# Gaurav14cs17/Bayer_Low_light_Image_Enhancement

Measured on AMD Instinct MI355X. Metric: megapixels/sec RawFormer-S 512x512 RAW->sRGB, higher is better.
Workload: dtype f32; 1 GPU; RawFormer-S(FLCA) dim=32, batch=8 of packed 4x512x512 synthetic Bayer per GPU; frames_per_gpu=8, variant=flca, weights=synthetic (seeded, random-init scale), parallelism=batch-sharded x1, device=AMD Radeon Graphics

## Files before the change

### bayer_low_light_image_enhancement_amd/build.py

```python
from __future__ import annotations

import os
import shutil
import subprocess
import sys
import tempfile
from concurrent.futures import ThreadPoolExecutor

HERE = os.path.dirname(os.path.abspath(__file__))
CSRC = os.path.join(HERE, "csrc")
LIB = os.path.join(CSRC, "librawformer_hip.so")
DIAG_LIB = os.path.join(CSRC, "librawformer_hip_diag.so")
DIAG_SOURCES = ["rf_block.hip", "rf_model.hip", "rf_gemm1x1.hip", "rf_fused.hip"]
SOURCES = ["rf_api.hip", "rf_model.hip", "rf_pack.hip", "rf_pointwise.hip", "rf_gemm1x1.hip",
           "rf_conv3x3.hip", "rf_attn.hip", "rf_flca.hip", "rf_fused.hip", "rf_block.hip", "rf_harness.hip", "rf_tokattn.hip", "rf_wfb.hip", "rf_upcat.hip", "rf_fft.hip", "rf_ffab.hip", "rf_truecolor.hip", "rf_train.hip", "rf_trainstep.hip"]
HEADERS = [os.path.join(CSRC, "rf_common.h"), os.path.join(CSRC, "rf_handle.h"), os.path.join(HERE, "..", "include", "rawformer_hip.h"),
           os.path.join(HERE, "isa_check.py")]
FLAGS = ["-O3", "-std=c++17", "-fPIC", "--offload-arch=gfx950", "-Wall", "-Wno-unused-function"]


def _hipcc() -> str:
    exe = shutil.which("hipcc") or "/opt/rocm/bin/hipcc"
    if not os.path.exists(exe):
        raise RuntimeError("hipcc not found: the RawFormer HIP library cannot be built here")
    return exe


def _run(cmd, cwd=None) -> str:
    r = subprocess.run(cmd, capture_output=True, text=True, cwd=cwd)
    if r.returncode != 0:
        raise RuntimeError("build step failed:\n" + " ".join(cmd) + "\n" + r.stdout + r.stderr)
    return r.stderr


def compile_source(src: str, obj: str, extra_flags=(), verbose: bool = False) -> int:
    from . import isa_check

    hipcc = _hipcc()
    llvm = isa_check.LLVM_BIN
    flags = [*FLAGS, *extra_flags]
    tmp = tempfile.mkdtemp(prefix="rf_build_")
    try:
        dev_s, dev_o, dev_co, fb = (os.path.join(tmp, n) for n in ("dev.s", "dev.o", "dev.co", "dev.hipfb"))
        warn = _run([hipcc, *flags, "--cuda-device-only", "-S", src, "-o", dev_s])
        text, nfix = isa_check.commute_vulnerable(open(dev_s).read())
        if nfix:
            open(dev_s, "w").write(text)
        _run([os.path.join(llvm, "clang"), "-target", "amdgcn-amd-amdhsa", "-mcpu=gfx950", "-c", dev_s, "-o", dev_o])
        _run([os.path.join(llvm, "lld"), "-flavor", "gnu", "-m", "elf64_amdgpu", "--no-undefined", "-shared", "-o", dev_co, dev_o])
        _run([os.path.join(llvm, "clang-offload-bundler"), "-type=o", "-bundle-align=4096",
              "-targets=host-x86_64-unknown-linux-gnu,hipv4-amdgcn-amd-amdhsa--gfx950", "-input=/dev/null", f"-input={dev_co}", f"-output={fb}"])
        _run([hipcc, *flags, "--cuda-host-only", "-c", src, "-Xclang", "-fcuda-include-gpubinary", "-Xclang", fb, "-o", obj])
    finally:
        shutil.rmtree(tmp, ignore_errors=True)
    if verbose:
        print(f"{os.path.basename(src)}: {nfix} packed-f32 operand-select instruction(s) commuted" + (("\n" + warn) if warn.strip() else ""), flush=True)
    return nfix


def _stale(target: str, deps) -> bool:
    if not os.path.exists(target):
        return True
    t = os.path.getmtime(target)
    return any(os.path.getmtime(d) > t for d in deps)


def build_library(force: bool = False, verbose: bool = False) -> str:
    hipcc = _hipcc()
    headers = HEADERS
    objs, jobs = [], []
    for src in SOURCES:
        s = os.path.join(CSRC, src)
        o = os.path.join(CSRC, src.replace(".hip", ".o"))
        objs.append(o)
        if force or _stale(o, [s] + headers):
            jobs.append((s, o))

    with ThreadPoolExecutor(max_workers=4) as ex:
        list(ex.map(lambda so: compile_source(so[0], so[1], verbose=verbose), jobs))
    if force or jobs or _stale(LIB, objs):
        _run([hipcc, "-shared", "-fPIC", "--offload-arch=gfx950", *objs, "-o", LIB])
    return LIB


def build_diag_library(force: bool = False, verbose: bool = False) -> str:
    build_library(force=force, verbose=verbose)
    hipcc = _hipcc()
    headers = HEADERS
    objs, rebuilt = [], False
    for src in SOURCES:
        s = os.path.join(CSRC, src)
        if src in DIAG_SOURCES:
            o = os.path.join(CSRC, src.replace(".hip", "_diag.o"))
            if force or _stale(o, [s] + headers):
                compile_source(s, o, extra_flags=["-DRF_DIAG"], verbose=verbose)
                rebuilt = True
        else:
            o = os.path.join(CSRC, src.replace(".hip", ".o"))
        objs.append(o)
    if force or rebuilt or _stale(DIAG_LIB, objs):
        r = subprocess.run([hipcc, "-shared", "-fPIC", "--offload-arch=gfx950", *objs, "-o", DIAG_LIB], capture_output=True, text=True)
        if r.returncode != 0:
            raise RuntimeError("hipcc link failed:\n" + r.stdout + r.stderr)
    return DIAG_LIB


if __name__ == "__main__":
    print(build_library(force="--force" in sys.argv, verbose=True))
    if "--diag" in sys.argv:
        print(build_diag_library(verbose=True))
```

### bayer_low_light_image_enhancement_amd/csrc/rf_api.hip

```cpp
#include <cstdarg>
#include <cstdio>
#include <cstring>
#include <map>
#include <string>
#include <vector>
#include "rf_common.h"

namespace rf {

static thread_local char g_err[512] = "";

void set_error(const char* fmt, ...) {
    va_list ap;
    va_start(ap, fmt);
    vsnprintf(g_err, sizeof(g_err), fmt, ap);
    va_end(ap);
}

int check_hip(hipError_t e, const char* what) {
    if (e == hipSuccess) return RF_OK;
    set_error("%s: %s", what, hipGetErrorString(e));
    return RF_E_DEVICE;
}

int check_launch(const char* what) { return check_hip(hipGetLastError(), what); }

struct ProfRec {
    std::string key;
    double flops, bytes;
    hipEvent_t e0, e1;
};
static bool g_prof_on = false;
static std::vector<ProfRec> g_prof;

ProfScope::ProfScope(hipStream_t st, const char* key, double flops, double bytes) : st_(st), rec_(-1) {
    if (!g_prof_on) return;
    ProfRec r;
    r.key = key;
    r.flops = flops;
    r.bytes = bytes;
    if (hipEventCreate(&r.e0) != hipSuccess || hipEventCreate(&r.e1) != hipSuccess) return;
    (void)hipEventRecord(r.e0, st);
    rec_ = (int)g_prof.size();
    g_prof.push_back(r);
}

bool profiling_active() { return g_prof_on; }

ProfScope::~ProfScope() {
    if (rec_ >= 0) (void)hipEventRecord(g_prof[rec_].e1, st_);
}

static const float kHaarInit[16] = {
    0.5f, 0.5f, 0.5f, 0.5f, -0.5f, 0.5f, -0.5f, 0.5f, -0.5f, -0.5f, 0.5f, 0.5f, 0.5f, -0.5f, -0.5f, 0.5f};
static const float kHaarOrtho[16] = {
    0.5f, 0.5f, 0.5f, 0.5f, 0.5f, -0.5f, 0.5f, -0.5f, 0.5f, 0.5f, -0.5f, -0.5f, 0.5f, -0.5f, -0.5f, 0.5f};

}

using namespace rf;

extern "C" {

const char* rf_last_error(void) { return g_err; }
int rf_version(void) { return 1; }

int rf_profile_begin(void) {
    for (auto& r : g_prof) { (void)hipEventDestroy(r.e0); (void)hipEventDestroy(r.e1); }
    g_prof.clear();
    g_prof_on = true;
    return RF_OK;
}

int rf_profile_end(char* json, size_t len) {
    g_prof_on = false;
    struct Agg { long n = 0; double ms = 0, flops = 0, bytes = 0; };
    std::map<std::string, Agg> agg;
    int rc = RF_OK;
    for (auto& r : g_prof) {
        float ms = 0.f;
        if (hipEventSynchronize(r.e1) != hipSuccess || hipEventElapsedTime(&ms, r.e0, r.e1) != hipSuccess) rc = RF_E_DEVICE;
        Agg& a = agg[r.key];
        a.n += 1; a.ms += ms; a.flops += r.flops; a.bytes += r.bytes;
        (void)hipEventDestroy(r.e0);
        (void)hipEventDestroy(r.e1);
    }
    g_prof.clear();
    if (rc) { set_error("rf_profile_end: event timing failed"); return rc; }
    std::string out = "[";
    bool first = true;
    for (auto& kv : agg) {
        char buf[512];
        snprintf(buf, sizeof(buf), "%s{\"kernel\": \"%s\", \"launches\": %ld, \"ms\": %.6f, \"flops\": %.6e, \"bytes\": %.6e}",
                 first ? "" : ", ", kv.first.c_str(), kv.second.n, kv.second.ms, kv.second.flops, kv.second.bytes);
        out += buf;
        first = false;
    }
    out += "]";
    RF_CHECK_ARG(json && out.size() + 1 <= len, "rf_profile_end: buffer of %zu bytes too small (need %zu)", len, out.size() + 1);
    memcpy(json, out.c_str(), out.size() + 1);
    return RF_OK;
}

int rf_pixel_unshuffle2(const float* in, float* out, int B, int C, int h, int w, void* stream) {
    RF_CHECK_ARG(in && out && B > 0 && C > 0 && h > 0 && w > 0, "pixel_unshuffle2: bad arguments");
    return launch_pixel_unshuffle2(in, out, B, C, h, w, (hipStream_t)stream);
}

int rf_pixel_shuffle2(const float* in, float* out, int B, int C, int h, int w, void* stream) {
    RF_CHECK_ARG(in && out && B > 0 && C > 0 && h > 0 && w > 0, "pixel_shuffle2: bad arguments");
    return launch_pixel_shuffle2(in, out, B, C, h, w, (hipStream_t)stream);
}

int rf_dwt_haar(const float* in, float* out, int B, int C, int h, int w, void* stream) {
    RF_CHECK_ARG(in && out && B > 0 && C > 0 && h > 0 && w > 0, "dwt_haar: bad arguments");
    return launch_dwt2x2(in, out, kHaarInit, 0, 1, B, C, h, w, 2 * h, 2 * w, (hipStream_t)stream);
}

int rf_idwt_haar(const float* in, float* out, int B, int C, int h, int w, void* stream) {
    RF_CHECK_ARG(in && out && B > 0 && C > 0 && h > 0 && w > 0, "idwt_haar: bad arguments");
    return launch_idwt2x2(in, out, kHaarInit, 0, 1, B, C, h, w, (hipStream_t)stream);
}

static void scaled_kernel(const float* k16, int norm, float out[16]) {
    for (int i = 0; i < 16; ++i) out[i] = norm ? k16[i] / 2.0f : k16[i];
}

int rf_dwt_custom(const float* in, float* out, const float* k16, int norm, int B, int C, int h, int w, void* stream) {
    RF_CHECK_ARG(in && out && k16 && B > 0 && C > 0 && h > 0 && w > 0, "dwt_custom: bad arguments");
    float k[16];
    scaled_kernel(k16, norm, k);
    return launch_dwt2x2(in, out, k, 1, 0, B, C, h, w, 2 * h, 2 * w, (hipStream_t)stream);
}

int rf_idwt_custom(const float* in, float* out, const float* k16, int norm, int B, int C, int h, int w, void* stream) {
    RF_CHECK_ARG(in && out && k16 && B > 0 && C > 0 && h > 0 && w > 0, "idwt_custom: bad arguments");
    float k[16];
    scaled_kernel(k16, norm, k);
    return launch_idwt2x2(in, out, k, 1, 0, B, C, h, w, (hipStream_t)stream);
}

int rf_haar_dwt(const float* in, float* out, int B, int C, int hin, int win, void* stream) {
    RF_CHECK_ARG(in && out && B > 0 && C > 0 && hin > 1 && win > 1, "haar_dwt: bad arguments");
    return launch_dwt2x2(in, out, kHaarOrtho, 0, 0, B, C, (hin + 1) / 2, (win + 1) / 2, hin, win, (hipStream_t)stream);
}

int rf_layernorm2d(const float* in, float* out, const float* weight, const float* bias, float eps,
                   int B, int C, int h, int w, void* stream) {
    RF_CHECK_ARG(in && out && weight && B > 0 && C > 0 && h > 0 && w > 0, "layernorm2d: bad arguments");
    return launch_layernorm2d(in, out, weight, bias, eps, B, C, h * w, (hipStream_t)stream);
}

int rf_conv1x1_scratch_bytes(int Cin_total, int Cout, size_t* bytes) {
    RF_CHECK_ARG(bytes && Cin_total > 0 && Cout > 0, "conv1x1_scratch_bytes: bad arguments");
    *bytes = (align_up(packed1x1_floats(Cin_total, Cout), 64) + packed1x1_b3_floats(Cin_total, Cout)) * sizeof(float);
    return RF_OK;
}

int rf_conv1x1(const float* in, const float* in2, float* out, const float* weight, const float* bias,
               const float* ln_w, const float* ln_b, const float* res, void* scratch,
               int B, int C1, int C2, int Cout, int h, int w, void* stream) {
    RF_CHECK_ARG(in && out && weight && scratch && aligned16(scratch), "conv1x1: bad arguments");
    hipStream_t st = (hipStream_t)stream;
    const int K = C1 + C2;
    RF_TRY(pack_1x1(weight, (float*)scratch, Cout, K, K, 1, st));
    float* w3 = (float*)scratch + align_up(packed1x1_floats(K, Cout), 64);
    RF_TRY(pack_1x1_b3(weight, w3, Cout, K, K, 1, st));
    Conv1x1Args a{};
    a.x1 = in; a.C1 = C1; a.x1_bstride = (int64_t)C1 * h * w;
    a.x2 = C2 ? in2 : nullptr; a.C2 = C2; a.x2_bstride = (int64_t)C2 * h * w;
    a.wp = (const float*)scratch; a.wp3 = w3; a.bias = bias; a.ln_w = ln_w; a.ln_b = ln_b; a.ln_eps = 1e-5f;
    a.res = res; a.res_bstride = (int64_t)Cout * h * w;
    a.out = out; a.out_bstride = (int64_t)Cout * h * w; a.Cout = Cout; a.B = B; a.P = h * w; a.w = w;
    return launch_conv1x1(a, st);
}

int rf_dwconv3x3(const float* in, float* out, const float* weight, const float* bias, int gelu,
                 int B, int C, int h, int w, void* stream) {
    RF_CHECK_ARG(in && out && weight && B > 0 && C > 0 && h > 0 && w > 0, "dwconv3x3: bad arguments");
    DwConvArgs a{};
    a.x = in; a.x_bstride = (int64_t)C * h * w; a.out = out; a.out_bstride = (int64_t)C * h * w;
    a.w = weight; a.bias = bias; a.B = B; a.C = C; a.h = h; a.w_ = w; a.gelu = gelu;
    return launch_dwconv3x3(a, (hipStream_t)stream);
}

int rf_conv3x3_scratch_bytes(int Cin, int Cout, size_t* bytes) {
    RF_CHECK_ARG(bytes && Cin > 0 && Cout > 0, "conv3x3_scratch_bytes: bad arguments");
    *bytes = packed3x3_floats(Cin, Cout) * sizeof(float);
    return RF_OK;
}

int rf_conv3x3(const float* in, float* out, const float* weight, const float* bias, void* scratch,
               int act, int store, int B, int Cin, int Cout, int h, int w, void* stream) {
    RF_CHECK_ARG(in && out && weight && scratch && aligned16(scratch), "conv3x3: bad arguments");
    hipStream_t st = (hipStream_t)stream;
    RF_TRY(pack_3x3(weight, (float*)scratch, Cout, Cin, st));
    Conv3x3Args a{};
    a.x = in; a.x_bstride = (int64_t)Cin * h * w; a.wp = (const float*)scratch; a.bias = bias;
    a.out = out; a.out_bstride = (int64_t)Cout * h * w; a.B = B; a.Cin = Cin; a.Cout = Cout; a.h = h; a.w = w;
    a.act = act; a.store = store;
    return launch_conv3x3(a, st);
}

int rf_convT2x2_scratch_bytes(int Cin, int Cout, size_t* bytes) {
    RF_CHECK_ARG(bytes && Cin > 0 && Cout > 0, "convT2x2_scratch_bytes: bad arguments");
    *bytes = packed1x1_floats(Cin, 4 * Cout) * sizeof(float);
    return RF_OK;
}

int rf_convT2x2(const float* in, float* out, const float* weight, const float* bias, void* scratch,
                int B, int Cin, int Cout, int h, int w, void* stream) {
    RF_CHECK_ARG(in && out && weight && scratch && aligned16(scratch), "convT2x2: bad arguments");
    hipStream_t st = (hipStream_t)stream;
    RF_TRY(pack_convT(weight, (float*)scratch, Cin, Cout, st));
    Conv1x1Args a{};
    a.x1 = in; a.C1 = Cin; a.x1_bstride = (int64_t)Cin * h * w; a.wp = (const float*)scratch; a.bias = bias;
    a.out = out; a.out_bstride = (int64_t)Cout * 4 * h * w; a.Cout = 4 * Cout; a.B = B; a.P = h * w; a.w = w; a.mode = 1;
    return launch_conv1x1(a, st);
}

struct AttnScratch {
    size_t wqkv, wqkv3, pre, qkv, partial, wfold, wfold3, total;
};
static int attn_scratch(int B, int C, int heads, int h, int w, AttnScratch* s) {
    const int P = h * w;
    int ns, sl;
    size_t pf;
    RF_TRY(gram_plan(B, C, heads, P, &ns, &sl, &pf));
    if (attn_mid_supported(C, heads, h, w)) {
        size_t pf2;
        attn_mid_plan(h, w, &ns, &pf2, B, C);
        if (pf2 > pf) pf = pf2;
    }
    size_t off = 0;
    auto take = [&](size_t f) { const size_t o = off; off += align_up(f, 64); return o; };
    s->wqkv = take(packed1x1_floats(C, 3 * C));
    s->wqkv3 = take(packed1x1_b3_floats(C, 3 * C));
    s->pre = take((size_t)B * 3 * C * P);
    s->qkv = take((size_t)B * 3 * C * P);
    s->partial = take(pf);
    s->wfold = take((size_t)B * packed1x1_floats(C, C));
    s->wfold3 = take((size_t)B * packed1x1_b3_floats(C, C));
    s->total = off;
    return RF_OK;
}

int rf_chan_attn_scratch_bytes(int B, int C, int heads, int h, int w, size_t* bytes) {
    RF_CHECK_ARG(bytes && B > 0 && C > 0 && heads > 0 && h > 0 && w > 0, "chan_attn_scratch_bytes: bad arguments");
    AttnScratch s;
    RF_TRY(attn_scratch(B, C, heads, h, w, &s));
    *bytes = s.total * sizeof(float);
    return RF_OK;
}

int rf_chan_attn(const float* in, float* out, const float* qkv_w, const float* qkv_b,
                 const float* dw_w, const float* dw_b, const float* temperature,
                 const float* proj_w, const float* proj_b, void* scratch,
                 int B, int C, int heads, int h, int w, void* stream) {
    RF_CHECK_ARG(in && out && qkv_w && dw_w && temperature && proj_w && scratch && aligned16(scratch), "chan_attn: bad arguments");
    hipStream_t st = (hipStream_t)stream;
    const int P = h * w;
    AttnScratch s;
    RF_TRY(attn_scratch(B, C, heads, h, w, &s));
    float* ws = (float*)scratch;
    RF_TRY(pack_1x1(qkv_w, ws + s.wqkv, 3 * C, C, C, 1, st));
    RF_TRY(pack_1x1_b3(qkv_w, ws + s.wqkv3, 3 * C, C, C, 1, st));
    Conv1x1Args q{};
    q.x1 = in; q.C1 = C; q.x1_bstride = (int64_t)C * P; q.wp = ws + s.wqkv; q.wp3 = ws + s.wqkv3; q.bias = qkv_b;
    q.out = ws + s.pre; q.out_bstride = (int64_t)3 * C * P; q.Cout = 3 * C; q.B = B; q.P = P; q.w = w;
    RF_TRY(launch_conv1x1(q, st));
    Conv1x1Args av{};
    int nslab = 0;
    if (attn_mid_supported(C, heads, h, w)) {
        size_t pf;
        RF_TRY(attn_mid_plan(h, w, &nslab, &pf, B, C));
        RF_TRY(launch_attn_mid(ws + s.pre, ws + s.qkv, ws + s.partial, nslab, dw_w, dw_b, B, C, h, w, st));
        av.x1 = ws + s.qkv; av.x1_bstride = (int64_t)C * P;
    } else {
        DwConvArgs d{};
        d.x = ws + s.pre; d.x_bstride = (int64_t)3 * C * P; d.out = ws + s.qkv; d.out_bstride = (int64_t)3 * C * P;
        d.w = dw_w; d.bias = dw_b; d.B = B; d.C = 3 * C; d.h = h; d.w_ = w;
        RF_TRY(launch_dwconv3x3(d, st));
        GramArgs g{};
        g.q = ws + s.qkv; g.k = ws + s.qkv + (size_t)C * P; g.bstride = (int64_t)3 * C * P;
        g.B = B; g.C = C; g.heads = heads; g.P = P; g.partial = ws + s.partial;
        size_t pf;
        RF_TRY(gram_plan(B, C, heads, P, &g.nslab, &g.slab, &pf));
        RF_TRY(launch_gram(g, st));
        nslab = g.nslab;
        av.x1 = ws + s.qkv + (size_t)2 * C * P; av.x1_bstride = (int64_t)3 * C * P;
    }
    RF_TRY(launch_attn_fold(ws + s.partial, nslab, temperature, proj_w, ws + s.wfold, ws + s.wfold3, B, C, heads, st));
    av.C1 = C;
    av.wp = ws + s.wfold; av.wp_bstride = (int64_t)packed1x1_floats(C, C); av.bias = proj_b;
    av.wp3 = ws + s.wfold3; av.wp3_bstride = (int64_t)packed1x1_b3_floats(C, C);
    av.out = out; av.out_bstride = (int64_t)C * P; av.Cout = C; av.B = B; av.P = P; av.w = w;
    return launch_conv1x1(av, st);
}

struct TbScratch { size_t wqkv, w1, w2, wqkv3, w13, w23, bufs, total; TbBufOffsets o; };
static void tb_scratch(int B, int C, int heads, int hc, int h, int w, TbScratch* s) {
    size_t off = 0;
    auto take = [&](size_t f) { const size_t r = off; off += align_up(f, 64); return r; };
    s->wqkv = take(packed1x1_floats(C, 3 * C));
    s->w1 = take(packed1x1_floats(C, hc));
    s->w2 = take(packed1x1_floats(hc, C));
    s->wqkv3 = take(packed1x1_b3_floats(C, 3 * C));
    s->w13 = take(packed1x1_b3_floats(C, hc));
    s->w23 = take(packed1x1_b3_floats(hc, C));
    s->bufs = off;
    s->total = off + transformer_scratch_floats(B, C, heads, hc, h, w, &s->o);
}

int rf_transformer_block_scratch_bytes(int B, int C, int heads, int ffn_expansion, int h, int w, size_t* bytes) {
    RF_CHECK_ARG(bytes && B > 0 && C > 0 && heads > 0 && C % heads == 0 && ffn_expansion > 0 && h > 0 && w > 0, "transformer_block_scratch_bytes: bad arguments");
    { int ns, sl; size_t pf; RF_TRY(gram_plan(B, C, heads, h * w, &ns, &sl, &pf)); }
    TbScratch s;
    tb_scratch(B, C, heads, C * ffn_expansion, h, w, &s);
    *bytes = s.total * sizeof(float);
    return RF_OK;
}

int rf_transformer_block(const float* in, float* out, const float* const* prm, void* scratch,
                         int B, int C, int heads, int ffn_expansion, int h, int w, void* stream) {
    RF_CHECK_ARG(in && out && prm && scratch && aligned16(scratch), "transformer_block: bad arguments");
    RF_CHECK_ARG(B > 0 && C % 4 == 0 && heads > 0 && C % heads == 0 && C / heads <= 64, "transformer_block: unsupported C=%d heads=%d", C, heads);
    for (int i = 0; i < 17; ++i) RF_CHECK_ARG(prm[i] != nullptr, "transformer_block: parameter %d is null", i);
    hipStream_t st = (hipStream_t)stream;
    const int hc = C * ffn_expansion;
    { int ns, sl; size_t pf; RF_TRY(gram_plan(B, C, heads, h * w, &ns, &sl, &pf)); }
    TbScratch s;
    tb_scratch(B, C, heads, hc, h, w, &s);
    float* ws = (float*)scratch;
    RF_TRY(pack_1x1(prm[3], ws + s.wqkv, 3 * C, C, C, 1, st));
    RF_TRY(pack_1x1(prm[11], ws + s.w1, hc, C, C, 1, st));
    RF_TRY(pack_1x1(prm[15], ws + s.w2, C, hc, hc, 1, st));
    RF_TRY(pack_1x1_b3(prm[3], ws + s.wqkv3, 3 * C, C, C, 1, st));
    RF_TRY(pack_1x1_b3(prm[11], ws + s.w13, hc, C, C, 1, st));
    RF_TRY(pack_1x1_b3(prm[15], ws + s.w23, C, hc, hc, 1, st));
    TbParams p{prm[0], prm[1], prm[2], ws + s.wqkv, prm[4], prm[5], prm[6], prm[7], prm[8],
               prm[9], prm[10], ws + s.w1, prm[12], prm[13], prm[14], ws + s.w2, prm[16],
               ws + s.wqkv3, ws + s.w13, ws + s.w23, 0};
    return run_transformer(p, in, out, ws + s.bufs, s.o, B, C, heads, hc, h, w, st);
}

int rf_flca_scratch_bytes(int B, int C, int h, int w, size_t* bytes) {
    RF_CHECK_ARG(bytes && B > 0 && C > 0 && h > 0 && w > 0, "flca_scratch_bytes: bad arguments");
    *bytes = (align_up((size_t)B * flca_nblk(h, w) * C, 64) + align_up((size_t)B * C, 64)) * sizeof(float);
    return RF_OK;
}

int rf_flca(const float* feat, const float* guide, float* out, const float* const* prm, void* scratch,
            int B, int C, int h, int w, void* stream) {
    RF_CHECK_ARG(feat && guide && out && prm && scratch && aligned16(scratch), "flca: bad arguments");
    for (int i = 0; i < 10; ++i) RF_CHECK_ARG(prm[i] != nullptr, "flca: parameter %d is null", i);
    hipStream_t st = (hipStream_t)stream;
    float* partial = (float*)scratch;
    float* ch = partial + align_up((size_t)B * flca_nblk(h, w) * C, 64);
    FlcaSpatialArgs a{};
    a.feat = feat; a.xs = out; a.guide = guide;
    a.alpha = prm[0]; a.beta = prm[1]; a.gamma = prm[2]; a.w_low = prm[3]; a.w_high = prm[4]; a.w_chr = prm[5];
    a.partial = partial; a.B = B; a.C = C; a.h = h; a.w = w; a.nblk = flca_nblk(h, w);
    RF_TRY(launch_flca_spatial(a, st));
    const int hid = C / 8 > 8 ? C / 8 : 8;
    RF_TRY(launch_flca_se(partial, a.nblk, h * w, prm[6], prm[7], prm[8], prm[9], hid, ch, B, C, st));
    return launch_scale_channels(out, ch, B, C, h * w, st);
}

int rf_guidance_scratch_bytes(int B, int H, int W, size_t* bytes) {
    RF_CHECK_ARG(bytes && B > 0 && H > 0 && W > 0, "guidance_scratch_bytes: bad arguments");
    *bytes = guidance_scratch_floats(B, H, W) * sizeof(float);
    return RF_OK;
}

int rf_flca_guidance(const float* packed, float* guide, void* scratch, int B, int H, int W, int hf, int wf, void* stream) {
    RF_CHECK_ARG(packed && guide && scratch && hf > 0 && wf > 0, "flca_guidance: bad arguments");
    hipStream_t st = (hipStream_t)stream;
    RF_TRY(launch_guidance_base(packed, 0, 0, (float*)scratch, B, H, W, st));
    return launch_guidance_level((const float*)scratch, guide, B, H, W, hf, wf, st);
}

int rf_upcat_scratch_bytes(int C, size_t* bytes) {
    RF_CHECK_ARG(bytes && C > 0 && C % 4 == 0, "upcat_scratch_bytes: bad arguments");
    *bytes = upcat_packed_floats(C) * sizeof(float);
    return RF_OK;
}

int rf_upcat(const float* x, const float* skip, float* out, const float* up_w, const float* up_b, const float* cr_w, const float* cr_b,
             void* scratch, int B, int C, int h, int w, void* stream) {
    RF_CHECK_ARG(x && skip && out && up_w && cr_w && scratch && aligned16(scratch), "upcat: bad arguments");
    hipStream_t st = (hipStream_t)stream;
    RF_TRY(pack_upcat(up_w, up_b, cr_w, cr_b, (float*)scratch, C, st));
    return launch_upcat(x, skip, out, (const float*)scratch, B, C, h, w, st);
}
}
```

### bayer_low_light_image_enhancement_amd/csrc/rf_common.h

```cpp
#pragma once
#include <hip/hip_runtime.h>
#include <stdint.h>
#include <stddef.h>
#include "../../include/rawformer_hip.h"

namespace rf {

typedef float f32x4 __attribute__((ext_vector_type(4)));

void set_error(const char* fmt, ...);
int check_hip(hipError_t e, const char* what);
int check_launch(const char* what);

#define RF_CHECK_ARG(cond, ...)            \
    do {                                   \
        if (!(cond)) {                     \
            rf::set_error(__VA_ARGS__);    \
            return RF_E_INVALID;           \
        }                                  \
    } while (0)

#define RF_TRY(expr)            \
    do {                        \
        const int rc_ = (expr); \
        if (rc_) return rc_;    \
    } while (0)

struct ProfScope {
    ProfScope(hipStream_t st, const char* key, double flops, double bytes);
    ~ProfScope();
    hipStream_t st_;
    int rec_;
};
bool profiling_active();

__device__ __forceinline__ float gelu_fast(float v) {
    const float t = __builtin_amdgcn_rcpf(fmaf(0.3275911f * 0.70710678118654752440f, fabsf(v), 1.0f));
    float p = fmaf(1.061405429f, t, -1.453152027f);
    p = fmaf(p, t, 1.421413741f);
    p = fmaf(p, t, -0.284496736f);
    p = fmaf(p, t, 0.254829592f);
    const float ex = __builtin_amdgcn_exp2f((v * v) * (-0.5f * 1.44269504088896340736f));
    const float q = (p * t) * ex;
    const float h = 0.5f * v;
    return h + fmaf(-fabsf(h), q, fabsf(h));
}

static inline int cdiv(int a, int b) { return (a + b - 1) / b; }
static inline size_t align_up(size_t v, size_t a) { return (v + a - 1) / a * a; }
static inline bool aligned16(const void* p) { return (reinterpret_cast<uintptr_t>(p) & 15) == 0; }

static inline size_t packed1x1_floats(int K, int Cout) { return (size_t)cdiv(K, 4) * cdiv(Cout, 16) * 64; }
static inline size_t packed3x3_floats(int Cin, int Cout) { return (size_t)cdiv(Cin, 8) * 2 * 18 * cdiv(Cout, 16) * 64; }

static inline size_t packed1x1_b3_floats(int K, int Cout) { return (size_t)cdiv(K, 32) * cdiv(Cout, 16) * 768; }
int pack_1x1_b3(const float* w, void* packed3, int Cout, int K, int64_t row_stride, int64_t col_stride, hipStream_t st);
#ifdef __HIPCC__
typedef unsigned u32x4 __attribute__((ext_vector_type(4)));
typedef __bf16 bf16x8 __attribute__((ext_vector_type(8)));
__device__ __forceinline__ void b3_split(float x, unsigned& p0, unsigned& p1, unsigned& p2) {
    p0 = __float_as_uint(x);
    const float r1 = x - __uint_as_float(p0 & 0xffff0000u);
    p1 = __float_as_uint(r1);
    p2 = __float_as_uint(r1 - __uint_as_float(p1 & 0xffff0000u));
}
__device__ __forceinline__ unsigned b3_pack(unsigned even_elem, unsigned odd_elem) {
    return __builtin_amdgcn_perm(odd_elem, even_elem, 0x07060302u);
}
__device__ __forceinline__ size_t b3_index(int NT, int co, int k, int piece) {
    const int lane = (co & 15) + 16 * ((k & 31) >> 3);
    return ((((size_t)(k >> 5) * NT + (co >> 4)) * 3 + piece) * 64 + lane) * 8 + (k & 7);
}
__device__ __forceinline__ void b3_store(unsigned short* dst, int NT, int co, int k, float v) {
    unsigned p0, p1, p2;
    b3_split(v, p0, p1, p2);
    dst[b3_index(NT, co, k, 0)] = (unsigned short)(p0 >> 16);
    dst[b3_index(NT, co, k, 1)] = (unsigned short)(p1 >> 16);
    dst[b3_index(NT, co, k, 2)] = (unsigned short)(p2 >> 16);
}
__device__ __forceinline__ f32x4 b3_mfma(const u32x4 (&a)[3], const u32x4 (&b)[3], f32x4 c) {
#define RF_B3(x) __builtin_bit_cast(bf16x8, x)
    c = __builtin_amdgcn_mfma_f32_16x16x32_bf16(RF_B3(a[2]), RF_B3(b[0]), c, 0, 0, 0);
    c = __builtin_amdgcn_mfma_f32_16x16x32_bf16(RF_B3(a[0]), RF_B3(b[2]), c, 0, 0, 0);
    c = __builtin_amdgcn_mfma_f32_16x16x32_bf16(RF_B3(a[1]), RF_B3(b[1]), c, 0, 0, 0);
    c = __builtin_amdgcn_mfma_f32_16x16x32_bf16(RF_B3(a[1]), RF_B3(b[0]), c, 0, 0, 0);
    c = __builtin_amdgcn_mfma_f32_16x16x32_bf16(RF_B3(a[0]), RF_B3(b[1]), c, 0, 0, 0);
    c = __builtin_amdgcn_mfma_f32_16x16x32_bf16(RF_B3(a[0]), RF_B3(b[0]), c, 0, 0, 0);
#undef RF_B3
    return c;
}
__device__ __forceinline__ void b3_mfma4(const u32x4 (&a)[3], const u32x4 (&b)[4][3], f32x4 (&c)[4]) {
#define RF_B3(x) __builtin_bit_cast(bf16x8, x)
#define RF_B3_TERM(ia, ib)                                                                                     \
    _Pragma("unroll") for (int g = 0; g < 4; ++g)                                                              \
        c[g] = __builtin_amdgcn_mfma_f32_16x16x32_bf16(RF_B3(a[ia]), RF_B3(b[g][ib]), c[g], 0, 0, 0);
    RF_B3_TERM(2, 0) RF_B3_TERM(0, 2) RF_B3_TERM(1, 1) RF_B3_TERM(1, 0) RF_B3_TERM(0, 1) RF_B3_TERM(0, 0)
#undef RF_B3_TERM
#undef RF_B3
}
#endif

int pack_1x1(const float* w, float* packed, int Cout, int K, int64_t row_stride, int64_t col_stride, hipStream_t st);
int pack_3x3(const float* w, float* packed, int Cout, int Cin, hipStream_t st);
int pack_convT(const float* w, float* packed, int Cin, int Cout, hipStream_t st);

struct PackDesc {
    const float* src; float* dst;
    int kind;
    int rows, cols;
    int64_t rs, cs;
    int flip;
};
constexpr int kPackBatch = 48;
struct PackBatch { PackDesc d[kPackBatch]; };
size_t pack_desc_floats(const PackDesc& d);
int launch_pack_batch(const PackDesc* d, int n, hipStream_t st);

size_t upcat_packed_floats(int C);
int pack_upcat(const float* up_w, const float* up_b, const float* cr_w, const float* cr_b, float* packed, int C, hipStream_t st);
bool upcat_supported(int C, int h, int w, const void* x, const void* skip, const void* out);
int launch_upcat(const float* x, const float* skip, float* out, const float* packed, int B, int C, int h, int w, hipStream_t st);

struct Conv1x1Args {
    const float* x1;
    const float* x2;
    int C1, C2;
    int64_t x1_bstride;
    int64_t x2_bstride;
    const float* x3;
    int C3;
    int64_t x3_bstride;
    const float* wp;
    int64_t wp_bstride;
    const void* wp3;
    int64_t wp3_bstride;
    const float* bias;
    const float* ln_w;
    const float* ln_b;
    float ln_eps;
    const float* res;
    int64_t res_bstride;
    float* out;
    int64_t out_bstride;
    int Cout;
    int B, P;
    int w;
    int mode;
    int act;
};
int launch_conv1x1(const Conv1x1Args& a, hipStream_t st);
bool conv1x1_ln_single_pass(const Conv1x1Args& a);

struct Conv3x3Args {
    const float* x;
    int64_t x_bstride;
    const float* wp;
    const float* bias;
    float* out;
    int64_t out_bstride;
    int B, Cin, Cout, h, w;
    int act;
    int store;
    int unshuffle_in;
    int clamp_in;
    int clamp_out;
    float* ks_scratch = nullptr;
    size_t ks_floats = 0;
};
int launch_conv3x3(const Conv3x3Args& a, hipStream_t st);
size_t conv3x3_ksplit_floats(int B, int Cout, int h, int w);
size_t conv3x3_ksplit_counter_bytes();

int launch_layernorm2d(const float* in, float* out, const float* w, const float* b, float eps,
                       int B, int C, int P, hipStream_t st);
struct DwConvArgs {
    const float* x; int64_t x_bstride;
    float* out; int64_t out_bstride;
    const float* w;
    const float* bias;
    int B, C, h, w_;
    int gelu;
    float* out2 = nullptr;
};
int launch_dwconv3x3(const DwConvArgs& a, hipStream_t st);
int launch_pixel_unshuffle2(const float* in, float* out, int B, int C, int h, int w, hipStream_t st);
int launch_pixel_shuffle2(const float* in, float* out, int B, int C, int h, int w, hipStream_t st);
int launch_dwt2x2(const float* in, float* out, const float k[16], int layout, int exact_haar,
                  int B, int C, int h, int w, int hin, int win, hipStream_t st);
int launch_idwt2x2(const float* in, float* out, const float k[16], int layout, int exact_haar,
                   int B, int C, int h, int w, hipStream_t st);

struct GramArgs {
    const float* q; const float* k;
    int64_t bstride;
    int B, C, heads, P;
    float* partial;
    int nslab, slab;
    int p_lo = 0, p_hi = 0;
};
int gram_plan(int B, int C, int heads, int P, int* nslab, int* slab, size_t* partial_floats);
int launch_gram(const GramArgs& a, hipStream_t st);
int launch_attn_fold(const float* partial, int nslab, const float* temperature, const float* w_out,
                     float* wp_out, void* wp3_out , int B, int C, int heads, hipStream_t st,
                     int log_temperature = 0);

bool fused_ffn_supported(int C, int hidden, int h, int w);
int launch_ffn_fused(const float* x, float* out, const float* ln_w, const float* ln_b, const void* w1p , const float* b1,
                     const float* wd, const float* bd, const float* w2p, const float* b2, int B, int C, int h, int w, hipStream_t st);
bool fused_attn_supported(int C, int heads, int h, int w);
int fused_attn_plan(int h, int w, int* nslab, size_t* partial_floats, int B, int C);
int launch_attn_front(const float* x, float* v, float* partial, int nslab, const float* ln_w, const float* ln_b,
                      const void* wp , const float* bq, const float* wd, const float* bd, int B, int C, int h, int w, hipStream_t st,
                      int ylo = 0, int yhi = 0 );

bool attn_mid_supported(int C, int heads, int h, int w);
int attn_mid_plan(int h, int w, int* nslab, size_t* partial_floats, int B, int C);
int launch_attn_mid(const float* qkv, float* v, float* partial, int nslab, const float* wd, const float* bd,
                    int B, int C, int h, int w, hipStream_t st, int ylo = 0, int yhi = 0);

struct TbParams {
    const float *ln1_w, *ln1_b, *temperature;
    const float *qkv_wp , *qkv_b, *qkv_dw_w, *qkv_dw_b, *proj_w , *proj_b;
    const float *ln2_w, *ln2_b, *pw1_wp , *pw1_b, *dw_w, *dw_b, *pw2_wp , *pw2_b;
    const void *qkv_wp3, *pw1_wp3, *pw2_wp3;
    int log_temperature;
    int ylo = 0, yhi = 0;
    void (*allreduce)(void* user, float* buf, size_t n, int op, void* stream) = nullptr;
    void* allreduce_user = nullptr;
    bool defer_pw2 = false;
};
bool transformer_ffn_is_fused(const TbParams& p, int C, int hc, int hh, int ww);
struct TbBufOffsets { size_t bufA, bufB, x1, partial, wfold, wfold3; };
size_t transformer_scratch_floats(int B, int C, int heads, int hc, int h, int w, TbBufOffsets* o);
int run_transformer(const TbParams& p, const float* in, float* out, float* ws, const TbBufOffsets& o,
                    int B, int C, int heads, int hc, int hh, int ww, hipStream_t st);

int launch_rfft2_polar(const float* in, float* mag, float* pha, float2* cscratch, int planes, int h, int w, hipStream_t st);
int launch_polar_irfft2(const float* mag, const float* pha, const float* res, float* out, float2* cscratch, int planes, int h, int w,
                        float lim, hipStream_t st);
int launch_clamp(const float* in, float* out, size_t n, float lo, float hi, hipStream_t st);

size_t tc_front_scratch_floats(int B, int H, int W, int levels);
int launch_tc_front(const float* in, int mosaic, const float* wb_gains, const float* color_matrix, const float* wp_c0, const float* b_c0,
                    const float* wp_c2, const float* b_c2, const float* wp_d0, const float* b_d0, const float* wp_d2, const float* b_d2,
                    float* scratch, int B, int H, int W, int levels, hipStream_t st);
int launch_tc_guide_level(const float* scratch, float* guide, int B, int H, int W, int levels, int hf, int wf, hipStream_t st);
int tc_front_outputs(const float* scratch, const float** y, const float** crcb, const float** rgb, int B, int H, int W, int levels);
int tc_nblk(int h, int w);
int launch_tc_spatial(const float* feat, float* xs, const float* guide, const float* w_col, const float* b_col, const float* w_low,
                      const float* b_low, const float* w_high, const float* b_high, int B, int C, int h, int w, hipStream_t st);
int launch_tc_residual(const float* xs, const float* r, float* x2, float* partial, int B, int C, int h, int w, hipStream_t st);
int launch_tc_color_head(float* x, const float* const* prm, int B, size_t P, hipStream_t st);

size_t gram2_partial_floats(int B, int Ca, int Cb, int h, int w, int ntap);
int launch_gram2(const float* a, int64_t a_bstride, int Ca, const float* b, int64_t b_bstride, int Cb, float* out, int ld, float* partial,
                 size_t partial_cap, int B, int h, int w, int ntap, int sy, int sx, int per_image, size_t out_istride, int accumulate, hipStream_t st,
                 float* db = nullptr ,
                 const float* b2 = nullptr, int64_t b2_bstride = 0, int Cb2 = 0 );
int launch_reduce_rows(const float* partial, float* out, int nrows, size_t n, int accumulate, hipStream_t st);
int chan_sum_nblk(int P);
int launch_chan_sum(const float* x, int64_t bstride, float* out, float* partial, int B, int C, int P, int accumulate, hipStream_t st);
size_t ln_bwd_partial_floats(int B, int C, int P);
bool ln_bwd_fused_shape(int C, int P);
int launch_ln_bwd(const float* x, const float* dy, const float* gamma, float* dx, float* dgb, float* partial,
                  int B, int C, int P, float eps, int accumulate_dx, int accumulate_w, hipStream_t st,
                  const float* res = nullptr, int64_t res_bstride = 0);
size_t dw_wgrad_partial_floats(int B, int C, int P);
int launch_dw_wgrad(const float* x, const float* dy, float* dw, float* db, float* partial, int B, int C, int h, int w, int accumulate, hipStream_t st);
int launch_ewise(const float* a, const float* b, float* out, size_t n, int mode, float slope, hipStream_t st);
int launch_split_halves(const float* src, float* a, float* b, int B, int C, int P, hipStream_t st);
int launch_flip3x3(const float* w, float* out, int Cout, int Cin, int dense, hipStream_t st);
int loss_nblk();
int launch_loss(const float* pred, const float* gt, float* grad, float* loss_out, float* partial, size_t n, int mode, float eps, hipStream_t st);
int launch_adam(float* p, const float* g, float* m, float* v, size_t n, float lr, float b1, float b2, float eps, float wd, int decoupled,
                int step, float gscale, hipStream_t st);

size_t flca_bwd_scratch_floats(int B, int C, int h, int w);
int launch_flca_backward(const float* feat, const float* guide, const float* xs, const float* dz, int64_t dz_bstride, const float* ch,
                         const float* pool_partial, int pool_nblk, const float* const* prm, float* const* grd, float* dfeat, int accumulate,
                         float* scratch, size_t scratch_floats, int B, int C, int h, int w, hipStream_t st);

size_t guidance_scratch_floats(int B, int H, int W);
int launch_guidance_base(const float* in, int mosaic, int clamp_in, float* scratch, int B, int H, int W, hipStream_t st,
                         void (*allreduce)(void*, float*, size_t, int, void*) = nullptr, void* allreduce_user = nullptr);
int launch_guidance_level(const float* scratch, float* guide, int B, int H, int W, int hf, int wf, hipStream_t st);
struct FlcaSpatialArgs {
    const float* feat; float* xs; const float* guide;
    const float* w_low; const float* w_high; const float* w_chr;
    const float* alpha; const float* beta; const float* gamma;
    float* partial;
    int B, C, h, w, nblk;
    int ylo = 0, yhi = 0;
};
int flca_nblk(int h, int w);
int launch_flca_spatial(const FlcaSpatialArgs& a, hipStream_t st);
int launch_flca_se(const float* partial, int nblk, int P, const float* se1_w, const float* se1_b,
                   const float* se3_w, const float* se3_b, int hidden, float* ch_out, int B, int C, hipStream_t st);
int launch_scale_channels(float* x, const float* ch, int B, int C, int P, hipStream_t st);
int launch_scale_channels_to(const float* in, float* out, const float* ch, int B, int C, int P, hipStream_t st);
int launch_flca_se_fold(const float* partial, int nblk, int P, const float* se1_w, const float* se1_b,
                        const float* se3_w, const float* se3_b, int hidden, const float* w_cr,
                        float* wp_out, void* wp3_out , float* ch_out, int B, int C, hipStream_t st,
                        const float* composed = nullptr , int hc = 0);
size_t tail_composed_floats(int C, int hc);
int pack_tail(const float* w_cr, const float* b_cr, const float* w2, const float* b2, float* composed, int C, int hc, hipStream_t st);
int launch_tail_fold(const float* w_cr, const float* ch , const float* composed, void* wp3_out, int B, int C, int hc,
                     hipStream_t st);

}
```

### bayer_low_light_image_enhancement_amd/csrc/rf_conv3x3.hip

```cpp
#include <cstdio>
#include <cstdlib>
#include "rf_common.h"

namespace rf {

static constexpr int KC = 8;
static constexpr int kKsCounters = 4096;
typedef unsigned u32x4 __attribute__((ext_vector_type(4)));

template <int NCO, int LOG2_RW, int RPW, int NWV, bool KS = false>
__global__ void __launch_bounds__(64 * NWV, (NWV >= 8 || NCO >= 3) ? 1 : 2) conv3x3_kernel(Conv3x3Args a, int ngroups, int tiles_x, int ntiles, int vec) {
    constexpr int NTHR = 64 * NWV;
    constexpr int TAPS = 18;
    constexpr int NM = 6;
    constexpr int RW = 1 << LOG2_RW;
    constexpr int TW = 64 / RW;
    constexpr int TH = NWV * RW * RPW;
    static_assert(RPW == 1 || RW == 1, "two row groups per wave only with one row per group");
    constexpr int RS = TW + 8;
    constexpr int PS = ((TH + 2) * RS + 63) / 64 * 64;
    constexpr int NIN = KC * (TH + 2) * (TW + 2);
    constexpr int EPT = (NIN + NTHR - 1) / NTHR;
    constexpr int NW4 = 2 * TAPS * NCO * 16;
    constexpr int WPT = (NW4 + NTHR - 1) / NTHR;
    constexpr int BUF = KC * PS + 2 * TAPS * NCO * 64;
    __shared__ __attribute__((aligned(16))) float lds[2 * BUF];
    __shared__ float bias_l[NCO * 16];

    const int tid = threadIdx.x;
    const int lane = tid & 63, wave = tid >> 6;
    const int j = lane & 15, kq = lane >> 4;
    const int rowj = j / (16 / RW), cg = j % (16 / RW);
    const int grp = blockIdx.x % ngroups;
    const int wg = blockIdx.x / ngroups;
    const int b = blockIdx.y;
    const int h = a.h, w = a.w;
    const int NT = (a.Cout + 15) >> 4;
    const int t0 = grp * NCO;
    const int nchunks_all = (a.Cin + KC - 1) / KC;
    const int ksplit = KS ? (int)gridDim.z : 1, kz = KS ? (int)blockIdx.z : 0;
    const int ch_lo = KS ? (int)((long)kz * nchunks_all / ksplit) : 0, ch_hi = KS ? (int)((long)(kz + 1) * nchunks_all / ksplit) : nchunks_all;
    const float* xb = a.x + (size_t)b * a.x_bstride;
    const size_t chunk_stride = a.unshuffle_in ? (size_t)(KC / 4) * 4 * h * w : (size_t)KC * h * w;

    constexpr unsigned OOB = 0x80000000u;
    int prc[EPT];
    short loff[EPT];
    static_assert(PS - (TH + 2) * RS >= 16, "plane padding holds the dummy slots");
    const int dummy = (tid & 7) * PS + (TH + 2) * RS + ((tid >> 3) & 15);
#pragma unroll
    for (int i = 0; i < EPT; ++i) {
        const int idx = tid + NTHR * i;
        const int c = idx % (TW + 2);
        const int r = (idx / (TW + 2)) % (TH + 2);
        const int cl = idx / ((TW + 2) * (TH + 2));
        prc[i] = idx < NIN ? (cl << 16) | (r << 8) | c : -1;
        loff[i] = (short)(idx < NIN ? cl * PS + r * RS + c : dummy);
    }
    unsigned wvoff[WPT];
#pragma unroll
    for (int i = 0; i < WPT; ++i) {
        const int idx = tid + NTHR * i;
        const int l4 = idx % 16;
        const int t = (idx / 16) % NCO;
        const int kt = idx / (16 * NCO);
        const bool ok = idx < NW4 && t0 + t < NT;
        wvoff[i] = ok ? (unsigned)(((kt * NT + t0 + t) * 64 + l4 * 4) * 4) : OOB;
    }
    const int w_chunk_bytes = 2 * TAPS * NT * 64 * 4;
    const size_t plane_bytes = (size_t)h * w * 4;

    unsigned voff[EPT];
    int x0 = 0, y0 = 0;
    auto plan_tile = [&](int tile) {
        const int tx = tile % tiles_x, ty = tile / tiles_x;
        x0 = tx * TW;
        y0 = ty * TH;
#pragma unroll
        for (int i = 0; i < EPT; ++i) {
            int e = prc[i];
            asm volatile("" : "+v"(e));
            const int cl = e >> 16;
            const int y = y0 - 1 + ((e >> 8) & 255), x = x0 - 1 + (e & 255);
            const bool ok = e >= 0 && (unsigned)y < (unsigned)h && (unsigned)x < (unsigned)w;
            const int off_m = ((cl >> 2) * 2 * h + 2 * y + ((cl >> 1) & 1)) * (2 * w) + 2 * x + (cl & 1);
            const int off_p = (cl * h + y) * w + x;
            voff[i] = ok ? (unsigned)(4 * (a.unshuffle_in ? off_m : off_p)) : OOB;
        }
    };
    float xin[EPT];
    float4 win[WPT];
    auto load_chunk = [&](int ch) {
        const int cl_lim = min(KC, a.Cin - ch * KC);
        const float* src = xb + (size_t)ch * chunk_stride;
        const __amdgpu_buffer_rsrc_t rx = __builtin_amdgcn_make_buffer_rsrc(
            const_cast<float*>(src), 0, (int)(a.unshuffle_in ? (size_t)(cl_lim / 4) * 4 * plane_bytes : (size_t)cl_lim * plane_bytes), 0x00020000);
        const __amdgpu_buffer_rsrc_t rw = __builtin_amdgcn_make_buffer_rsrc(
            const_cast<float*>(a.wp) + (size_t)ch * (w_chunk_bytes / 4), 0, w_chunk_bytes, 0x00020000);
#pragma unroll
        for (int i = 0; i < EPT; ++i) xin[i] = __uint_as_float(__builtin_amdgcn_raw_buffer_load_b32(rx, (int)voff[i], 0, 0));
#pragma unroll
        for (int i = 0; i < WPT; ++i) {
            const u32x4 v = __builtin_amdgcn_raw_buffer_load_b128(rw, (int)wvoff[i], 0, 0);
            win[i] = make_float4(__uint_as_float(v.x), __uint_as_float(v.y), __uint_as_float(v.z), __uint_as_float(v.w));
        }
    };
    auto store_chunk = [&](int buf) {
        float* li = lds + buf * BUF;
        float* lw = li + KC * PS;
#pragma unroll
        for (int i = 0; i < EPT; ++i) {
            float v = xin[i];
            if (a.clamp_in) v = fminf(fmaxf(v, 0.f), 1.f);
            li[loff[i]] = v;
        }
#pragma unroll
        for (int i = 0; i < WPT; ++i) {
            const int idx = tid + NTHR * i;
            if (idx < NW4) *reinterpret_cast<float4*>(lw + idx * 4) = win[i];
        }
    };

    f32x4 acc[RPW][NCO][NM];

    const int nwg = gridDim.x / ngroups;
    int tile = wg;
    const int tile_end = ntiles;
    if (tile >= tile_end) return;
    if (tid < NCO * 16) {
        const int co = 16 * t0 + tid;
        bias_l[tid] = (a.bias && co < a.Cout) ? a.bias[co] : 0.f;
    }
    plan_tile(tile);
    load_chunk(ch_lo);
    store_chunk(0);
    __syncthreads();
    int buf = 0;
    float* outb = a.out + (size_t)b * a.out_bstride;
    for (; tile < tile_end; tile += nwg) {
        const int ex0 = x0, ey0 = y0;
#pragma unroll
        for (int rr = 0; rr < RPW; ++rr)
#pragma unroll
            for (int t = 0; t < NCO; ++t)
#pragma unroll
                for (int g = 0; g < NM; ++g) acc[rr][t][g] = (f32x4){0.f, 0.f, 0.f, 0.f};
        for (int ch = ch_lo; ch < ch_hi; ++ch) {
            const bool last = ch + 1 == ch_hi;
            const bool more = !last || tile + nwg < tile_end;
            const int nch = last ? ch_lo : ch + 1;
            if (last && more) plan_tile(tile + nwg);
            if (more) load_chunk(nch);
            const float* lds_in = lds + buf * BUF;
            const float* lds_w = lds_in + KC * PS;
            const int nks = (a.Cin - ch * KC > 4) ? 2 : 1;
#pragma unroll
            for (int ks = 0; ks < 2; ++ks) {
                if (ks >= nks) break;
                const float* lp = lds_in + (ks * 4 + kq) * PS + (wave * RW * RPW + rowj) * RS + 4 * cg;
#pragma unroll
                for (int ir = 0; ir < RPW + 2; ++ir) {
                    const float4 lo = *reinterpret_cast<const float4*>(lp + ir * RS);
                    const float4 hi = *reinterpret_cast<const float4*>(lp + ir * RS + 4);
                    float d[NM];
                    {
                        const float p = fmaf(-4.f, lo.z, hi.x), q = fmaf(-4.f, lo.y, lo.w);
                        const float c2 = hi.x - lo.z, e2 = lo.w - lo.y;
                        d[0] = fmaf(4.f, lo.x, fmaf(-5.f, lo.z, hi.x));
                        d[1] = p + q; d[2] = p - q;
                        d[3] = fmaf(2.f, e2, c2); d[4] = fmaf(-2.f, e2, c2);
                        d[5] = fmaf(4.f, lo.y, fmaf(-5.f, lo.w, hi.y));
                    }
#pragma unroll
                    for (int rr = 0; rr < RPW; ++rr) {
                        const int dy = ir - rr;
                        if (dy < 0 || dy > 2) continue;
#pragma unroll
                        for (int j4 = 0; j4 < TAPS / 3; ++j4) {
                            const float* wl = lds_w + ((ks * TAPS + dy * (TAPS / 3) + j4) * NCO) * 64 + lane;
#pragma unroll
                            for (int t = 0; t < NCO; ++t) {
                                acc[rr][t][j4] = __builtin_amdgcn_mfma_f32_16x16x4f32(wl[t * 64], d[j4], acc[rr][t][j4], 0, 0, 0);
                            }
                        }
                    }
                }
            }
            if (more) store_chunk(buf ^ 1);
            __syncthreads();
            buf ^= 1;
        }

    int kq_ = kq;
    asm volatile("" : "+v"(kq_));
    const int x = ex0 + 4 * cg;
    auto transform = [&](int rr, int t, float (&u)[4][4]) {
        const f32x4* mm = acc[rr][t];
#pragma unroll
        for (int r = 0; r < 4; ++r) {
            const float s12 = mm[1][r] + mm[2][r], d12 = mm[1][r] - mm[2][r], s34 = mm[3][r] + mm[4][r], d34 = mm[3][r] - mm[4][r];
            u[r][0] = (mm[0][r] + s12) + s34;
            u[r][1] = fmaf(2.f, d34, d12);
            u[r][2] = fmaf(4.f, s34, s12);
            u[r][3] = fmaf(8.f, d34, d12) + mm[5][r];
        }
    };
    auto finish = [&](int t, float (&v)[4][4]) {
#pragma unroll
        for (int r = 0; r < 4; ++r) {
            const float bs = bias_l[16 * t + 4 * kq_ + r];
#pragma unroll
            for (int g = 0; g < 4; ++g) {
                float u = v[r][g] + bs;
                if (a.act == 1) u = u > 0.f ? u : 0.2f * u;
                else if (a.act == 2) u = fmaxf(u, 0.f);
                else if (a.act == 3) u = gelu_fast(u);
                else if (a.act == 4) u = 1.0f - 2.0f * __builtin_amdgcn_rcpf(1.0f + __expf(2.0f * u));
                if (a.clamp_out) u = fminf(fmaxf(u, 0.f), 1.f);
                v[r][g] = u;
            }
        }
    };
    auto store_tile = [&](int t, int y, const float (&v)[4][4]) {
        const int cobase = 16 * (t0 + t) + 4 * kq_;
        if (a.store == 0) {
#pragma unroll
            for (int r = 0; r < 4; ++r) {
                const int co = cobase + r;
                if (co >= a.Cout) continue;
                float* o = outb + ((size_t)co * h + y) * w + x;
                if (vec) {
                    *reinterpret_cast<float4*>(o) = make_float4(v[r][0], v[r][1], v[r][2], v[r][3]);
                } else {
#pragma unroll
                    for (int g = 0; g < 4; ++g)
                        if (x + g < w) o[g] = v[r][g];
                }
            }
        } else if (a.store == 1) {
            const int h2 = h >> 1, w2 = w >> 1;
#pragma unroll
            for (int r = 0; r < 4; ++r) {
                const int co = cobase + r;
                if (co >= a.Cout) continue;
                float* o = outb + (((size_t)(4 * co + 2 * (y & 1))) * h2 + (y >> 1)) * w2 + (x >> 1);
                const size_t ps = (size_t)h2 * w2;
                if (vec) {
                    *reinterpret_cast<float2*>(o) = make_float2(v[r][0], v[r][2]);
                    *reinterpret_cast<float2*>(o + ps) = make_float2(v[r][1], v[r][3]);
                } else {
#pragma unroll
                    for (int g = 0; g < 4; ++g)
                        if (x + g < w) o[(size_t)(g & 1) * ps + (g >> 1)] = v[r][g];
                }
            }
        } else {
            if (cobase >= a.Cout) return;
            const int c = cobase >> 2;
            float* op = outb + (size_t)c * 4 * h * w;
            const int w2 = 2 * w;
            if (vec) {
#pragma unroll
                for (int i = 0; i < 2; ++i) {
                    float* row = op + (size_t)(2 * y + i) * w2 + 2 * x;
                    *reinterpret_cast<float4*>(row) = make_float4(v[2 * i][0], v[2 * i + 1][0], v[2 * i][1], v[2 * i + 1][1]);
                    *reinterpret_cast<float4*>(row + 4) = make_float4(v[2 * i][2], v[2 * i + 1][2], v[2 * i][3], v[2 * i + 1][3]);
                }
            } else {
#pragma unroll
                for (int g = 0; g < 4; ++g)
                    if (x + g < w) {
#pragma unroll
                        for (int r = 0; r < 4; ++r)
                            op[(size_t)(2 * y + (r >> 1)) * w2 + 2 * (x + g) + (r & 1)] = v[r][g];
                    }
            }
        }
    };
    if constexpr (!KS) {
#pragma unroll
        for (int rr = 0; rr < RPW; ++rr) {
            const int y = ey0 + (wave * RPW + rr) * RW + rowj;
            if (y >= h || x >= w) continue;
#pragma unroll
            for (int t = 0; t < NCO; ++t) {
                if (t0 + t >= NT) break;
                float v[4][4];
                transform(rr, t, v);
                finish(t, v);
                store_tile(t, y, v);
            }
        }
    } else {
        unsigned* counter = reinterpret_cast<unsigned*>(a.ks_scratch) + ((size_t)b * ntiles + tile) * ngroups + grp;
        float* part = a.ks_scratch + kKsCounters;
        const size_t split_stride = (size_t)a.B * a.Cout * h * w;
        float* mine = part + (size_t)kz * split_stride + (size_t)b * a.Cout * h * w;
#pragma unroll
        for (int rr = 0; rr < RPW; ++rr) {
            const int y = ey0 + (wave * RPW + rr) * RW + rowj;
            if (y >= h || x >= w) continue;
#pragma unroll
            for (int t = 0; t < NCO; ++t) {
                if (t0 + t >= NT) break;
                float v[4][4];
                transform(rr, t, v);
#pragma unroll
                for (int r = 0; r < 4; ++r) {
                    const int co = 16 * (t0 + t) + 4 * kq_ + r;
                    if (co < a.Cout) *reinterpret_cast<float4*>(mine + ((size_t)co * h + y) * w + x) = make_float4(v[r][0], v[r][1], v[r][2], v[r][3]);
                }
            }
        }
        __shared__ unsigned ticket;
        __builtin_amdgcn_fence(__ATOMIC_RELEASE, "agent");
        __syncthreads();
        if (tid == 0) ticket = atomicAdd(counter, 1u);
        __syncthreads();
        if (ticket != (unsigned)(ksplit - 1)) return;
        if (tid == 0) *counter = 0u;
        __builtin_amdgcn_fence(__ATOMIC_ACQUIRE, "agent");
#pragma unroll
        for (int rr = 0; rr < RPW; ++rr) {
            const int y = ey0 + (wave * RPW + rr) * RW + rowj;
            if (y >= h || x >= w) continue;
#pragma unroll
            for (int t = 0; t < NCO; ++t) {
                if (t0 + t >= NT) break;
                float v[4][4];
#pragma unroll
                for (int r = 0; r < 4; ++r) {
                    const int co = 16 * (t0 + t) + 4 * kq_ + r;
                    float4 sum = make_float4(0.f, 0.f, 0.f, 0.f);
                    if (co < a.Cout) {
                        const float* src = part + (size_t)b * a.Cout * h * w + ((size_t)co * h + y) * w + x;
                        for (int z = 0; z < ksplit; ++z) {
                            const float4 pz = *reinterpret_cast<const float4*>(src + (size_t)z * split_stride);
                            sum.x += pz.x; sum.y += pz.y; sum.z += pz.z; sum.w += pz.w;
                        }
                    }
                    v[r][0] = sum.x; v[r][1] = sum.y; v[r][2] = sum.z; v[r][3] = sum.w;
                }
                finish(t, v);
                store_tile(t, y, v);
            }
        }
        return;
    }
    }
}

size_t conv3x3_ksplit_counter_bytes() { return (size_t)kKsCounters * sizeof(float); }
size_t conv3x3_ksplit_floats(int B, int Cout, int h, int w) {
    return ((long)B * h * w <= 16384) ? (size_t)kKsCounters + (size_t)8 * B * Cout * h * w : 0;
}

static int ksplit_for(const Conv3x3Args& a, int ntiles, int ngroups, int vec, const dim3& grid) {
    if (!a.ks_scratch || !vec || !aligned16(a.ks_scratch)) return 1;
    const long total = (long)ntiles * ngroups * a.B;
    const int nchunks = cdiv(a.Cin, KC);
    if (total > 64 || total > kKsCounters || nchunks < 8 || (long)grid.x != (long)ngroups * ntiles) return 1;
    int S = nchunks / 4;
    if (S > 8) S = 8;
    while (S > 1 && total * S > 256) --S;
    if (S < 2 || (size_t)kKsCounters + (size_t)S * a.B * a.Cout * a.h * a.w > a.ks_floats) return 1;
    return S;
}

template <int NCO>
static void launch_rw(const Conv3x3Args& a, int ngroups, int vec, bool small, hipStream_t st) {
    const int lrw = a.w > 32 ? 0 : (a.w > 16 ? 1 : 2);
    constexpr int RPWB = NCO <= 2 ? 2 : 1;
    auto grid_for_tiles = [&](int ntiles) {
        const long total = (long)ntiles * ngroups * a.B;
        const int wgs = cdiv(ntiles, (int)((total + 255) / 256));
        return dim3((unsigned)(ngroups * wgs), (unsigned)a.B);
    };
    if (small && lrw == 0) {
        const int txs = cdiv(a.w, 64), ntiles = txs * cdiv(a.h, 4);
        dim3 grid = grid_for_tiles(ntiles);
        const int S = ksplit_for(a, ntiles, ngroups, vec, grid);
        grid.z = (unsigned)S;
        if (S > 1) conv3x3_kernel<NCO, 0, 1, 4, true><<<grid, 256, 0, st>>>(a, ngroups, txs, ntiles, vec);
        else conv3x3_kernel<NCO, 0, 1, 4><<<grid, 256, 0, st>>>(a, ngroups, txs, ntiles, vec);
    } else if (NCO == 1 && lrw == 0 && a.h >= 16) {
        const int txs = cdiv(a.w, 64), ntiles = txs * cdiv(a.h, 16);
        conv3x3_kernel<1, 0, 1, 16><<<grid_for_tiles(ntiles), 1024, 0, st>>>(a, ngroups, txs, ntiles, vec);
    } else if (lrw == 0 && a.h >= 8 * RPWB) {
        const int txs = cdiv(a.w, 64), ntiles = txs * cdiv(a.h, 8 * RPWB);
        conv3x3_kernel<NCO, 0, RPWB, 8><<<grid_for_tiles(ntiles), 512, 0, st>>>(a, ngroups, txs, ntiles, vec);
    } else if (lrw == 0 && a.h >= 8) {
        const int txs = cdiv(a.w, 64), ntiles = txs * cdiv(a.h, 8);
        conv3x3_kernel<NCO, 0, 1, 8><<<grid_for_tiles(ntiles), 512, 0, st>>>(a, ngroups, txs, ntiles, vec);
    } else {
        const int txs = cdiv(a.w, 64 >> lrw), ntiles = txs * cdiv(a.h, 4 << lrw);
        dim3 grid = grid_for_tiles(ntiles);
        const int S = ksplit_for(a, ntiles, ngroups, vec, grid);
        grid.z = (unsigned)S;
        if (S > 1) {
            if (lrw == 0) conv3x3_kernel<NCO, 0, 1, 4, true><<<grid, 256, 0, st>>>(a, ngroups, txs, ntiles, vec);
            else if (lrw == 1) conv3x3_kernel<NCO, 1, 1, 4, true><<<grid, 256, 0, st>>>(a, ngroups, txs, ntiles, vec);
            else conv3x3_kernel<NCO, 2, 1, 4, true><<<grid, 256, 0, st>>>(a, ngroups, txs, ntiles, vec);
        } else if (lrw == 0) conv3x3_kernel<NCO, 0, 1, 4><<<grid, 256, 0, st>>>(a, ngroups, txs, ntiles, vec);
        else if (lrw == 1) conv3x3_kernel<NCO, 1, 1, 4><<<grid, 256, 0, st>>>(a, ngroups, txs, ntiles, vec);
        else conv3x3_kernel<NCO, 2, 1, 4><<<grid, 256, 0, st>>>(a, ngroups, txs, ntiles, vec);
    }
}

int launch_conv3x3(const Conv3x3Args& a, hipStream_t st) {
    RF_CHECK_ARG(a.B > 0 && a.B <= 65535 && a.Cin > 0 && a.Cout > 0 && a.h > 0 && a.w > 0, "conv3x3: bad sizes");
    RF_CHECK_ARG(a.store == 0 || (a.store == 1 && a.h % 2 == 0 && a.w % 2 == 0) || (a.store == 2 && a.Cout % 4 == 0),
                 "conv3x3: store mode %d incompatible with Cout=%d h=%d w=%d", a.store, a.Cout, a.h, a.w);
    RF_CHECK_ARG(!a.unshuffle_in || a.Cin == 4, "conv3x3: the packed-mosaic input path takes exactly 4 channels");
    RF_CHECK_ARG((double)a.Cin * a.h * a.w * 4.0 < 2.0e9, "conv3x3: image too large for 32-bit gather offsets");
    const int NT = cdiv(a.Cout, 16);
    int nco = 4;
    if (NT % 4 != 0) nco = (NT % 3 == 0) ? 3 : (NT % 2 == 0 ? 2 : (NT == 1 ? 1 : 4));
    bool small = false;
    if (a.w > 32 && a.h >= 8) {
        const long big = (long)cdiv(a.w, 64) * cdiv(a.h, nco <= 2 ? 16 : 8) * cdiv(NT, nco) * a.B;
        if (big < 128) {
            small = true;
            const long t4 = (long)cdiv(a.w, 64) * cdiv(a.h, 4) * a.B;
            while (nco > 1 && t4 * cdiv(NT, nco) < 192) nco = (nco == 4 || nco == 2) ? nco / 2 : 1;
        }
    }
    const int ngroups = cdiv(NT, nco);
    const int vec = (a.w % 4 == 0) && aligned16(a.out) && (a.out_bstride % 4 == 0);
    char key[64];
    {
        const int lrw = a.w > 32 ? 0 : (a.w > 16 ? 1 : 2), rpwb = nco <= 2 ? 2 : 1;
        const int wide = lrw == 0 && a.h >= 8;
        snprintf(key, sizeof(key), "conv3x3_kernel<%d, %d, %d, %d>", nco, lrw, (wide && a.h >= 8 * rpwb) ? rpwb : 1, wide ? 8 : 4);
        if (nco == 1 && lrw == 0 && a.h >= 16) snprintf(key, sizeof(key), "conv3x3_kernel<1, 0, 1, 16>");
        if (small) snprintf(key, sizeof(key), "conv3x3_kernel<%d, 0, 1, 4>", nco);
    }
    const double px = (double)a.B * a.h * a.w;
    ProfScope prof(st, key, 18.0 * a.Cin * a.Cout * px, 4.0 * px * (a.Cin + a.Cout));
    switch (nco) {
        case 4: launch_rw<4>(a, ngroups, vec, small, st); break;
        case 3: launch_rw<3>(a, ngroups, vec, small, st); break;
        case 2: launch_rw<2>(a, ngroups, vec, small, st); break;
        default: launch_rw<1>(a, ngroups, vec, small, st); break;
    }
    return check_launch("conv3x3");
}

}
```

### bayer_low_light_image_enhancement_amd/csrc/rf_handle.h

```cpp
#pragma once
#include <string>
#include <unordered_map>
#include <vector>
#include "rf_common.h"

struct Param {
    std::string name;
    int64_t shape[4];
    int ndim;
    const float* ptr;
    size_t numel() const {
        size_t n = 1;
        for (int i = 0; i < ndim; ++i) n *= (size_t)shape[i];
        return n;
    }
};

enum PackKind { PK_1x1, PK_3x3, PK_CONVT, PK_1x1_B3 };
struct PackItem {
    int param;
    PackKind kind;
    size_t offset;
    size_t floats;
};

struct SideStream {
    hipStream_t stream = nullptr;
    hipEvent_t ev_fork = nullptr, ev_join = nullptr;
    bool failed = false;
    bool pending = false;
    int forks = 0;
    hipStream_t get(hipStream_t st);
    int fork(hipStream_t st, hipStream_t side);
    int join(hipStream_t st, hipStream_t side);
    void join_pending(hipStream_t st);
    void destroy();
};

struct SideJoinGuard {
    SideStream& s;
    hipStream_t st;
    SideJoinGuard(SideStream& s_, hipStream_t st_) : s(s_), st(st_) { s.forks = 0; }
    ~SideJoinGuard() { s.join_pending(st); }
};

struct rf_handle {
    rf_config cfg;
    std::vector<Param> params;
    std::unordered_map<std::string, int> index;
    std::vector<PackItem> packs;
    std::unordered_map<std::string, int> pack_index;
    std::unordered_map<std::string, int> pack3_index;
    size_t packed_floats = 0;
    size_t upcat_offset[3] = {0, 0, 0};
    size_t tail_offset[8] = {0, 0, 0, 0, 0, 0, 0, 0}, tail3_offset[8] = {0, 0, 0, 0, 0, 0, 0, 0};
    const float* packed = nullptr;
    std::vector<size_t> flat_offset;
    size_t flat_floats = 0;
    int shard_y_lo = 0, shard_y_hi = 0, shard_total_rows = 0;
    void (*shard_allreduce)(void* user, float* buf, size_t n, int op, void* stream) = nullptr;
    void* shard_user = nullptr;
    SideStream side;
    void (*grad_ready)(void* user, size_t offset, size_t count, void* stream) = nullptr;
    void* grad_ready_user = nullptr;
};


inline const float* rf_param_ptr(const rf_handle* h, const std::string& name) { return h->params[h->index.at(name)].ptr; }
inline int rf_param_index(const rf_handle* h, const std::string& name) { return h->index.at(name); }
```

### bayer_low_light_image_enhancement_amd/csrc/rf_model.hip

```cpp
#include <string>
#include <unordered_map>
#include <vector>
#include <cstring>
#include <cstdlib>
#include "rf_common.h"

using namespace rf;

#include "rf_handle.h"

namespace {

void add_param(rf_handle* h, const std::string& name, std::initializer_list<int64_t> shape) {
    Param p;
    p.name = name;
    p.ndim = (int)shape.size();
    int i = 0;
    for (auto s : shape) p.shape[i++] = s;
    for (; i < 4; ++i) p.shape[i] = 1;
    p.ptr = nullptr;
    h->index[name] = (int)h->params.size();
    h->params.push_back(p);
}

void add_pack(rf_handle* h, const std::string& name, PackKind kind) {
    const int pi = h->index.at(name);
    const Param& p = h->params[pi];
    PackItem it;
    it.param = pi;
    it.kind = kind;
    it.offset = h->packed_floats;
    if (kind == PK_1x1) it.floats = packed1x1_floats((int)p.shape[1], (int)p.shape[0]);
    else if (kind == PK_3x3) it.floats = packed3x3_floats((int)p.shape[1], (int)p.shape[0]);
    else if (kind == PK_1x1_B3) it.floats = packed1x1_b3_floats((int)p.shape[1], (int)p.shape[0]);
    else it.floats = packed1x1_floats((int)p.shape[0], 4 * (int)p.shape[1]);
    h->packed_floats += align_up(it.floats, 64);
    (kind == PK_1x1_B3 ? h->pack3_index : h->pack_index)[name] = (int)h->packs.size();
    h->packs.push_back(it);
}

bool tail_composable(int C, int hc) { return C % 32 == 0 && hc % 32 == 0 && hc > 0; }

void add_stage(rf_handle* h, int i, int C, int heads) {
    const rf_config& cfg = h->cfg;
    const std::string pre = "conv_tran" + std::to_string(i) + ".";
    if (cfg.variant == RF_VARIANT_TRUECOLOR) {
        const std::string f = pre + "FLCA.";
        const int hid = C / 8 > 8 ? C / 8 : 8;
        add_param(h, f + "color_attention.0.weight", {C, 5, 3, 3});
        add_param(h, f + "color_attention.0.bias", {C});
        add_param(h, f + "low_attn.0.weight", {C, 1, 3, 3});
        add_param(h, f + "low_attn.0.bias", {C});
        add_param(h, f + "high_attn.0.weight", {C, 1, 3, 3});
        add_param(h, f + "high_attn.0.bias", {C});
        add_param(h, f + "se.1.weight", {hid, C, 1, 1});
        add_param(h, f + "se.1.bias", {hid});
        add_param(h, f + "se.3.weight", {C, hid, 1, 1});
        add_param(h, f + "se.3.bias", {C});
        add_param(h, f + "res_proj.0.weight", {C, C, 1, 1});
        add_param(h, f + "res_proj.0.bias", {C});
        add_param(h, f + "res_proj.2.weight", {C, C, 1, 1});
        add_param(h, f + "res_proj.2.bias", {C});
        for (const char* n : {"res_proj.0.weight", "res_proj.2.weight"}) {
            add_pack(h, f + n, PK_1x1);
            add_pack(h, f + n, PK_1x1_B3);
        }
    } else if (cfg.variant == RF_VARIANT_FLCA) {
        const std::string f = pre + "FLCA.";
        const int hid = C / 8 > 8 ? C / 8 : 8;
        add_param(h, f + "alpha", {});
        add_param(h, f + "beta", {});
        add_param(h, f + "gamma", {});
        add_param(h, f + "low_attn.0.weight", {C, 1, 3, 3});
        add_param(h, f + "high_attn.0.weight", {C, 1, 3, 3});
        add_param(h, f + "chroma_attn.0.weight", {C, 2, 3, 3});
        add_param(h, f + "se.1.weight", {hid, C, 1, 1});
        add_param(h, f + "se.1.bias", {hid});
        add_param(h, f + "se.3.weight", {C, hid, 1, 1});
        add_param(h, f + "se.3.bias", {C});
    } else {
        add_param(h, pre + "conv.weight", {C, C, 3, 3});
        add_param(h, pre + "conv.bias", {C});
        add_pack(h, pre + "conv.weight", PK_3x3);
    }
    const std::string t = pre + "Transformer.";
    const int hc = C * cfg.ffn_expansion;
    add_param(h, t + "norm1.body.weight", {C});
    add_param(h, t + "norm1.body.bias", {C});
    add_param(h, t + (cfg.variant == RF_VARIANT_TRUECOLOR ? "attn.log_temperature" : "attn.temperature"), {heads, 1, 1});
    add_param(h, t + "attn.qkv.weight", {3 * C, C, 1, 1});
    add_param(h, t + "attn.qkv.bias", {3 * C});
    add_param(h, t + "attn.qkv_dwconv.weight", {3 * C, 1, 3, 3});
    add_param(h, t + "attn.qkv_dwconv.bias", {3 * C});
    add_param(h, t + "attn.project_out.weight", {C, C, 1, 1});
    add_param(h, t + "attn.project_out.bias", {C});
    add_param(h, t + "norm2.body.weight", {C});
    add_param(h, t + "norm2.body.bias", {C});
    add_param(h, t + "ffn.pointwise1.weight", {hc, C, 1, 1});
    add_param(h, t + "ffn.pointwise1.bias", {hc});
    add_param(h, t + "ffn.depthwise.weight", {hc, 1, 3, 3});
    add_param(h, t + "ffn.depthwise.bias", {hc});
    add_param(h, t + "ffn.pointwise2.weight", {C, hc, 1, 1});
    add_param(h, t + "ffn.pointwise2.bias", {C});
    add_param(h, pre + "channel_reduce.weight", {C, 2 * C, 1, 1});
    add_param(h, pre + "channel_reduce.bias", {C});
    add_param(h, pre + "Conv_out.weight", {C, C, 3, 3});
    add_param(h, pre + "Conv_out.bias", {C});
    add_pack(h, t + "attn.qkv.weight", PK_1x1);
    add_pack(h, t + "ffn.pointwise1.weight", PK_1x1);
    add_pack(h, t + "ffn.pointwise2.weight", PK_1x1);
    add_pack(h, t + "attn.qkv.weight", PK_1x1_B3);
    add_pack(h, t + "ffn.pointwise1.weight", PK_1x1_B3);
    add_pack(h, t + "ffn.pointwise2.weight", PK_1x1_B3);
    if (cfg.variant == RF_VARIANT_PLAIN) {
        add_pack(h, pre + "channel_reduce.weight", PK_1x1);
        add_pack(h, pre + "channel_reduce.weight", PK_1x1_B3);
    }
    if (tail_composable(C, hc)) {
        h->tail_offset[i] = h->packed_floats;
        h->packed_floats += align_up(tail_composed_floats(C, hc), 64);
        if (cfg.variant == RF_VARIANT_PLAIN) {
            h->tail3_offset[i] = h->packed_floats;
            h->packed_floats += align_up(packed1x1_b3_floats(2 * C + hc, C), 64);
        }
    }
    add_pack(h, pre + "Conv_out.weight", PK_3x3);
}

const float* P(const rf_handle* h, const std::string& name) { return h->params[h->index.at(name)].ptr; }
const float* PK(const rf_handle* h, const std::string& name) { return h->packed + h->packs[h->pack_index.at(name)].offset; }
const float* PK3(const rf_handle* h, const std::string& name) { return h->packed + h->packs[h->pack3_index.at(name)].offset; }

struct Plan {
    size_t total = 0;
    size_t gscratch, guide[4], skip[3], tA, tB, tU, bufA, bufB, x1, trans, xs, cr;
    size_t gram_partial, wfold_attn, wfold_cr, wfold_attn3, wfold_cr3, flca_partial, ch;
    size_t ks, ks_floats;
    int guide_planes;
};

size_t take(Plan& p, size_t floats) {
    const size_t off = p.total;
    p.total += align_up(floats, 64);
    return off;
}

int make_plan(const rf_handle* h, int B, int H, int W, Plan& p) {
    const rf_config& c = h->cfg;
    const size_t U0 = (size_t)B * c.dim * H * W;
    const bool tc = c.variant == RF_VARIANT_TRUECOLOR;
    const int levels = c.flca_levels > 0 ? c.flca_levels : 2;
    p.guide_planes = tc ? 7 : 4;
    p.gscratch = take(p, tc ? tc_front_scratch_floats(B, H, W, levels) : guidance_scratch_floats(B, H, W));
    for (int l = 0; l < 4; ++l) p.guide[l] = take(p, (size_t)B * p.guide_planes * (H >> l) * (W >> l));
    for (int l = 0; l < 3; ++l) p.skip[l] = take(p, U0 >> l);
    p.tA = take(p, U0);
    p.tB = take(p, U0);
    p.tU = take(p, U0);
    const size_t wide = (size_t)(c.ffn_expansion > 3 ? c.ffn_expansion : 3);
    p.bufA = take(p, wide * U0);
    p.bufB = take(p, wide * U0);
    p.x1 = take(p, U0);
    p.trans = take(p, U0);
    p.xs = take(p, U0);
    p.cr = take(p, U0);
    size_t gp = 0, wa = 0, wc = 0, fp = 0, wa3 = 0, wc3 = 0;
    for (int l = 0; l < 4; ++l) {
        const int C = c.dim << l, Pl = (H >> l) * (W >> l);
        int ns, sl;
        size_t pf;
        const int rc = gram_plan(B, C, c.heads[l], Pl, &ns, &sl, &pf);
        if (rc) return rc;
        if (pf > gp) gp = pf;
        if (fused_attn_supported(C, c.heads[l], H >> l, W >> l)) {
            size_t pf2;
            fused_attn_plan(H >> l, W >> l, &ns, &pf2, B, C);
            if (pf2 > gp) gp = pf2;
        }
        if (attn_mid_supported(C, c.heads[l], H >> l, W >> l)) {
            size_t pf2;
            attn_mid_plan(H >> l, W >> l, &ns, &pf2, B, C);
            if (pf2 > gp) gp = pf2;
        }
        const size_t a = (size_t)B * packed1x1_floats(C, C), cr = (size_t)B * packed1x1_floats(2 * C, C);
        if (a > wa) wa = a;
        if (cr > wc) wc = cr;
        const int hcl = C * c.ffn_expansion;
        const size_t a3 = (size_t)B * packed1x1_b3_floats(C, C),
                     cr3 = (size_t)B * packed1x1_b3_floats(tail_composable(C, hcl) ? 2 * C + hcl : 2 * C, C);
        if (a3 > wa3) wa3 = a3;
        if (cr3 > wc3) wc3 = cr3;
        const size_t f = (size_t)B * (tc ? tc_nblk(H >> l, W >> l) : flca_nblk(H >> l, W >> l)) * C;
        if (f > fp) fp = f;
    }
    p.gram_partial = take(p, gp);
    p.wfold_attn = take(p, wa);
    p.wfold_cr = take(p, wc);
    p.wfold_attn3 = take(p, wa3);
    p.wfold_cr3 = take(p, wc3);
    p.flca_partial = take(p, fp);
    p.ch = take(p, (size_t)B * (c.dim << 3));
    p.ks_floats = 0;
    for (int l = 0; l < 4; ++l) {
        const size_t f = conv3x3_ksplit_floats(B, c.dim << l, H >> l, W >> l);
        if (f > p.ks_floats) p.ks_floats = f;
    }
    p.ks = take(p, p.ks_floats);
    return RF_OK;
}

int run_stage(rf_handle* h, int i, int lvl, const float* in, float* out, float* ws, const Plan& p,
              int B, int H, int W, hipStream_t st, hipStream_t side) {
    const rf_config& cfg = h->cfg;
    const int C = cfg.dim << lvl, hh = H >> lvl, ww = W >> lvl, Pn = hh * ww, heads = cfg.heads[lvl];
    const int hc = C * cfg.ffn_expansion;
    const std::string pre = "conv_tran" + std::to_string(i) + ".", t = pre + "Transformer.";
    float* trans = ws + p.trans;
    float* xs = ws + p.xs;
    float* crb = ws + p.cr;

    TbParams tp{};
    tp.ln1_w = P(h, t + "norm1.body.weight"); tp.ln1_b = P(h, t + "norm1.body.bias");
    if (cfg.variant != RF_VARIANT_TRUECOLOR) tp.temperature = P(h, t + "attn.temperature");
    tp.qkv_wp = PK(h, t + "attn.qkv.weight"); tp.qkv_b = P(h, t + "attn.qkv.bias");
    tp.qkv_dw_w = P(h, t + "attn.qkv_dwconv.weight"); tp.qkv_dw_b = P(h, t + "attn.qkv_dwconv.bias");
    tp.proj_w = P(h, t + "attn.project_out.weight"); tp.proj_b = P(h, t + "attn.project_out.bias");
    tp.ln2_w = P(h, t + "norm2.body.weight"); tp.ln2_b = P(h, t + "norm2.body.bias");
    tp.pw1_wp = PK(h, t + "ffn.pointwise1.weight"); tp.pw1_b = P(h, t + "ffn.pointwise1.bias");
    tp.dw_w = P(h, t + "ffn.depthwise.weight"); tp.dw_b = P(h, t + "ffn.depthwise.bias");
    tp.pw2_wp = PK(h, t + "ffn.pointwise2.weight"); tp.pw2_b = P(h, t + "ffn.pointwise2.bias");
    tp.qkv_wp3 = PK3(h, t + "attn.qkv.weight"); tp.pw1_wp3 = PK3(h, t + "ffn.pointwise1.weight"); tp.pw2_wp3 = PK3(h, t + "ffn.pointwise2.weight");
    if (cfg.variant == RF_VARIANT_TRUECOLOR) { tp.temperature = P(h, t + "attn.log_temperature"); tp.log_temperature = 1; }
    const bool sharded = h->shard_allreduce != nullptr;
    const int ylo = sharded ? h->shard_y_lo >> lvl : 0, yhi = sharded ? h->shard_y_hi >> lvl : 0;
    const int P_pool = sharded ? (h->shard_total_rows >> lvl) * ww : Pn;
    if (sharded) { tp.ylo = ylo; tp.yhi = yhi; tp.allreduce = h->shard_allreduce; tp.allreduce_user = h->shard_user; }
    TbBufOffsets to{p.bufA, p.bufB, p.x1, p.gram_partial, p.wfold_attn, p.wfold_attn3};
    bool compose = h->tail_offset[i] != 0 && Pn % 4 == 0 && !transformer_ffn_is_fused(tp, C, hc, hh, ww);
#ifdef RF_DIAG
    if (getenv("RF_NO_COMPOSE") || getenv("RF_NO_B3")) compose = false;
#endif
    tp.defer_pw2 = compose;
    const float* composed = compose ? h->packed + h->tail_offset[i] : nullptr;
    if (cfg.variant == RF_VARIANT_TRUECOLOR) RF_TRY(run_transformer(tp, in, trans, ws, to, B, C, heads, hc, hh, ww, st));
    else RF_TRY(h->side.fork(st, side));

    Conv1x1Args r{};
    r.x1 = xs; r.C1 = C; r.x1_bstride = (int64_t)C * Pn;
    r.x2 = trans; r.C2 = C; r.x2_bstride = (int64_t)C * Pn;
    r.bias = P(h, pre + "channel_reduce.bias");
    r.out = crb; r.out_bstride = (int64_t)C * Pn; r.Cout = C; r.B = B; r.P = Pn; r.w = ww;
    if (cfg.variant == RF_VARIANT_TRUECOLOR) {
        const std::string f = pre + "FLCA.";
        RF_TRY(launch_tc_spatial(in, xs, ws + p.guide[lvl], P(h, f + "color_attention.0.weight"), P(h, f + "color_attention.0.bias"),
                                 P(h, f + "low_attn.0.weight"), P(h, f + "low_attn.0.bias"), P(h, f + "high_attn.0.weight"),
                                 P(h, f + "high_attn.0.bias"), B, C, hh, ww, st));
        Conv1x1Args r0{};
        r0.x1 = xs; r0.C1 = C; r0.x1_bstride = (int64_t)C * Pn; r0.wp = PK(h, f + "res_proj.0.weight"); r0.wp3 = PK3(h, f + "res_proj.0.weight");
        r0.bias = P(h, f + "res_proj.0.bias"); r0.out = crb; r0.out_bstride = (int64_t)C * Pn; r0.Cout = C; r0.B = B; r0.P = Pn; r0.w = ww; r0.act = 2;
        RF_TRY(launch_conv1x1(r0, st));
        Conv1x1Args r2 = r0;
        r2.x1 = crb; r2.wp = PK(h, f + "res_proj.2.weight"); r2.wp3 = PK3(h, f + "res_proj.2.weight"); r2.bias = P(h, f + "res_proj.2.bias");
        r2.out = ws + p.bufA; r2.act = 0;
        RF_TRY(launch_conv1x1(r2, st));
        RF_TRY(launch_tc_residual(xs, ws + p.bufA, xs, ws + p.flca_partial, B, C, hh, ww, st));
        const int hid = C / 8 > 8 ? C / 8 : 8;
        RF_TRY(launch_flca_se_fold(ws + p.flca_partial, tc_nblk(hh, ww), Pn, P(h, f + "se.1.weight"), P(h, f + "se.1.bias"),
                                   P(h, f + "se.3.weight"), P(h, f + "se.3.bias"), hid, P(h, pre + "channel_reduce.weight"),
                                   ws + p.wfold_cr, ws + p.wfold_cr3, ws + p.ch, B, C, st, composed, hc));
        r.wp = ws + p.wfold_cr; r.wp_bstride = (int64_t)packed1x1_floats(2 * C, C);
        r.wp3 = ws + p.wfold_cr3; r.wp3_bstride = (int64_t)packed1x1_b3_floats(compose ? 2 * C + hc : 2 * C, C);
    } else if (cfg.variant == RF_VARIANT_FLCA) {
        const std::string f = pre + "FLCA.";
        FlcaSpatialArgs s{};
        s.feat = in; s.xs = xs; s.guide = ws + p.guide[lvl];
        s.w_low = P(h, f + "low_attn.0.weight"); s.w_high = P(h, f + "high_attn.0.weight"); s.w_chr = P(h, f + "chroma_attn.0.weight");
        s.alpha = P(h, f + "alpha"); s.beta = P(h, f + "beta"); s.gamma = P(h, f + "gamma");
        s.partial = ws + p.flca_partial; s.B = B; s.C = C; s.h = hh; s.w = ww; s.nblk = flca_nblk(hh, ww);
        s.ylo = ylo; s.yhi = yhi;
        RF_TRY(launch_flca_spatial(s, side));
        if (sharded) h->shard_allreduce(h->shard_user, s.partial, (size_t)B * s.nblk * C, 0, (void*)side);
        const int hid = C / 8 > 8 ? C / 8 : 8;
        RF_TRY(launch_flca_se_fold(s.partial, s.nblk, P_pool, P(h, f + "se.1.weight"), P(h, f + "se.1.bias"),
                                   P(h, f + "se.3.weight"), P(h, f + "se.3.bias"), hid, P(h, pre + "channel_reduce.weight"),
                                   ws + p.wfold_cr, ws + p.wfold_cr3, ws + p.ch, B, C, side, composed, hc));
        r.wp = ws + p.wfold_cr; r.wp_bstride = (int64_t)packed1x1_floats(2 * C, C);
        r.wp3 = ws + p.wfold_cr3; r.wp3_bstride = (int64_t)packed1x1_b3_floats(compose ? 2 * C + hc : 2 * C, C);
    } else {
        Conv3x3Args cb{};
        cb.x = in; cb.x_bstride = (int64_t)C * Pn; cb.wp = PK(h, pre + "conv.weight"); cb.bias = P(h, pre + "conv.bias");
        cb.out = xs; cb.out_bstride = (int64_t)C * Pn; cb.B = B; cb.Cin = C; cb.Cout = C; cb.h = hh; cb.w = ww;
        cb.act = cfg.branch_lrelu ? 1 : 0;
        RF_TRY(launch_conv3x3(cb, side));
        r.wp = PK(h, pre + "channel_reduce.weight");
        r.wp3 = compose ? h->packed + h->tail3_offset[i] : PK3(h, pre + "channel_reduce.weight");
    }
    if (cfg.variant != RF_VARIANT_TRUECOLOR) {
        RF_TRY(run_transformer(tp, in, trans, ws, to, B, C, heads, hc, hh, ww, st));
        RF_TRY(h->side.join(st, side));
    }
    if (compose) {
        r.wp = nullptr;
        r.x2 = ws + p.x1;
        r.x3 = ws + p.bufB; r.C3 = hc; r.x3_bstride = (int64_t)hc * Pn;
        r.bias = composed + (size_t)C * hc;
    }
    RF_TRY(launch_conv1x1(r, st));

    Conv3x3Args co{};
    co.x = crb; co.x_bstride = (int64_t)C * Pn; co.wp = PK(h, pre + "Conv_out.weight"); co.bias = P(h, pre + "Conv_out.bias");
    co.out = out; co.out_bstride = (int64_t)C * Pn; co.B = B; co.Cin = C; co.Cout = C; co.h = hh; co.w = ww; co.act = 1;
    if (p.ks_floats) { co.ks_scratch = ws + p.ks; co.ks_floats = p.ks_floats; }
    RF_TRY(launch_conv3x3(co, st));
    return RF_OK;
}

}

hipStream_t SideStream::get(hipStream_t st) {
    if (failed || profiling_active()) return st;
    if (!stream &&
        (hipStreamCreateWithFlags(&stream, hipStreamNonBlocking) != hipSuccess ||
         hipEventCreateWithFlags(&ev_fork, hipEventDisableTiming) != hipSuccess ||
         hipEventCreateWithFlags(&ev_join, hipEventDisableTiming) != hipSuccess)) {
        (void)hipGetLastError();
        destroy();
        failed = true;
        return st;
    }
    return stream;
}

int SideStream::fork(hipStream_t st, hipStream_t side) {
    if (side == st) return RF_OK;
    pending = true;
    ++forks;
    RF_TRY(check_hip(hipEventRecord(ev_fork, st), "side stream fork (record)"));
    RF_TRY(check_hip(hipStreamWaitEvent(side, ev_fork, 0), "side stream fork (wait)"));
#ifdef RF_DIAG
    const char* n = getenv("RF_FAIL_FORK");
    if (n && forks == atoi(n)) {
        set_error("RF_FAIL_FORK=%s: injected failure of fork %d", n, forks);
        return RF_E_DEVICE;
    }
#endif
    return RF_OK;
}

int SideStream::join(hipStream_t st, hipStream_t side) {
    if (side == st) return RF_OK;
    RF_TRY(check_hip(hipEventRecord(ev_join, side), "side stream join (record)"));
    RF_TRY(check_hip(hipStreamWaitEvent(st, ev_join, 0), "side stream join (wait)"));
    pending = false;
    return RF_OK;
}

void SideStream::destroy() {
    if (stream) (void)hipStreamDestroy(stream);
    if (ev_fork) (void)hipEventDestroy(ev_fork);
    if (ev_join) (void)hipEventDestroy(ev_join);
    stream = nullptr;
    ev_fork = ev_join = nullptr;
}

void SideStream::join_pending(hipStream_t st) {
    if (!pending) return;
    if (hipEventRecord(ev_join, stream) != hipSuccess || hipStreamWaitEvent(st, ev_join, 0) != hipSuccess) {
        (void)hipGetLastError();
        (void)hipStreamSynchronize(stream);
    }
    pending = false;
}

extern "C" {

int rf_create(const rf_config* cfg, rf_handle** out) {
    RF_CHECK_ARG(cfg && out, "rf_create: null argument");
    RF_CHECK_ARG(cfg->dim > 0 && cfg->dim % 8 == 0, "rf_create: dim=%d must be a positive multiple of 8", cfg->dim);
    RF_CHECK_ARG(cfg->inp_channels == 1, "rf_create: inp_channels=%d (only the 1-channel Bayer mosaic is supported)", cfg->inp_channels);
    RF_CHECK_ARG(cfg->out_channels > 0 && cfg->ffn_expansion > 0, "rf_create: bad out_channels / ffn_expansion");
    RF_CHECK_ARG(cfg->variant == RF_VARIANT_FLCA || cfg->variant == RF_VARIANT_PLAIN || cfg->variant == RF_VARIANT_TRUECOLOR,
                 "rf_create: unknown variant %d", cfg->variant);
    RF_CHECK_ARG(cfg->flca_levels >= 0 && cfg->flca_levels <= 3, "rf_create: flca_levels=%d (1..3, 0 = default 2)", cfg->flca_levels);
    RF_CHECK_ARG(cfg->variant != RF_VARIANT_TRUECOLOR || cfg->out_channels == 3, "rf_create: the TrueColor colour head is defined for 3 output channels");
    for (int l = 0; l < 4; ++l) {
        const int C = cfg->dim << l;
        RF_CHECK_ARG(cfg->heads[l] > 0 && C % cfg->heads[l] == 0 && C / cfg->heads[l] <= 64,
                     "rf_create: heads[%d]=%d incompatible with %d channels (head size must divide and be <= 64)", l, cfg->heads[l], C);
        int ns, sl;
        size_t pf;
        RF_TRY(gram_plan(1, C, cfg->heads[l], 256, &ns, &sl, &pf));
    }
    rf_handle* h = new rf_handle();
    h->cfg = *cfg;
    const int d = cfg->dim;
    if (cfg->variant == RF_VARIANT_TRUECOLOR) {
        add_param(h, "bayer_processor.wb_gains", {4});
        add_param(h, "bayer_processor.color_matrix", {3, 4});
        add_param(h, "bayer_processor.demosaic_refine.0.weight", {32, 3, 3, 3});
        add_param(h, "bayer_processor.demosaic_refine.0.bias", {32});
        add_param(h, "bayer_processor.demosaic_refine.2.weight", {3, 32, 3, 3});
        add_param(h, "bayer_processor.demosaic_refine.2.bias", {3});
        add_param(h, "bayer_processor.chroma_extractor.0.weight", {16, 4, 3, 3});
        add_param(h, "bayer_processor.chroma_extractor.0.bias", {16});
        add_param(h, "bayer_processor.chroma_extractor.2.weight", {2, 16, 3, 3});
        add_param(h, "bayer_processor.chroma_extractor.2.bias", {2});
        for (const char* n : {"demosaic_refine.0.weight", "demosaic_refine.2.weight", "chroma_extractor.0.weight", "chroma_extractor.2.weight"})
            add_pack(h, std::string("bayer_processor.") + n, PK_3x3);
    }
    add_param(h, "embedding.weight", {d, 4 * cfg->inp_channels, 3, 3});
    add_param(h, "embedding.bias", {d});
    add_pack(h, "embedding.weight", PK_3x3);
    for (int i = 1; i <= 3; ++i) {
        const int C = d << (i - 1);
        add_stage(h, i, C, cfg->heads[i - 1]);
        const std::string n = "down" + std::to_string(i) + ".body.0.weight";
        add_param(h, n, {C / 2, C, 3, 3});
        add_pack(h, n, PK_3x3);
    }
    add_stage(h, 4, d * 8, cfg->heads[3]);
    for (int i = 1; i <= 3; ++i) {
        const int lvl = 3 - i, C = d << lvl;
        const std::string u = "up" + std::to_string(i), r = "channel_reduce" + std::to_string(i);
        add_param(h, u + ".weight", {2 * C, C, 2, 2});
        add_param(h, u + ".bias", {C});
        add_param(h, r + ".weight", {C, 2 * C, 1, 1});
        add_param(h, r + ".bias", {C});
        add_pack(h, u + ".weight", PK_CONVT);
        add_pack(h, r + ".weight", PK_1x1);
        h->upcat_offset[i - 1] = h->packed_floats;
        h->packed_floats += align_up(upcat_packed_floats(C), 64);
        add_stage(h, 4 + i, C, cfg->heads[lvl]);
    }
    add_param(h, "conv_out.weight", {4 * cfg->out_channels, d, 3, 3});
    add_param(h, "conv_out.bias", {4 * cfg->out_channels});
    add_pack(h, "conv_out.weight", PK_3x3);
    if (cfg->variant == RF_VARIANT_TRUECOLOR) {
        add_param(h, "color_correction.gamma_param", {});
        add_param(h, "color_correction.color_transform.0.weight", {64, 3, 1, 1});
        add_param(h, "color_correction.color_transform.0.bias", {64});
        add_param(h, "color_correction.color_transform.2.weight", {3, 64, 1, 1});
        add_param(h, "color_correction.color_transform.2.bias", {3});
        add_param(h, "color_correction.tone_curve.0.weight", {32, 1, 1, 1});
        add_param(h, "color_correction.tone_curve.0.bias", {32});
        add_param(h, "color_correction.tone_curve.2.weight", {1, 32, 1, 1});
        add_param(h, "color_correction.tone_curve.2.bias", {1});
    }
    for (const Param& q : h->params) {
        h->flat_offset.push_back(h->flat_floats);
        h->flat_floats += align_up(q.numel(), 4);
    }
    *out = h;
    return RF_OK;
}

void rf_destroy(rf_handle* h) {
    if (!h) return;
    h->side.destroy();
    delete h;
}

int rf_param_count(const rf_handle* h) { return h ? (int)h->params.size() : RF_E_INVALID; }

int rf_param_info(const rf_handle* h, int index, const char** name, int64_t shape[4], int* ndim) {
    RF_CHECK_ARG(h && index >= 0 && index < (int)h->params.size(), "rf_param_info: index %d out of range", index);
    const Param& p = h->params[index];
    if (name) *name = p.name.c_str();
    if (shape) std::memcpy(shape, p.shape, sizeof(p.shape));
    if (ndim) *ndim = p.ndim;
    return RF_OK;
}

int rf_set_param(rf_handle* h, const char* name, const float* dev_ptr, const int64_t* shape, int ndim) {
    RF_CHECK_ARG(h && name && dev_ptr, "rf_set_param: null argument");
    auto it = h->index.find(name);
    if (it == h->index.end()) {
        set_error("rf_set_param: unexpected key '%s'", name);
        return RF_E_MISSING;
    }
    Param& p = h->params[it->second];
    size_t n = 1;
    for (int i = 0; i < ndim; ++i) n *= (size_t)shape[i];
    bool same = n == p.numel();
    if (same && ndim == p.ndim)
        for (int i = 0; i < ndim; ++i) same = same && shape[i] == p.shape[i];
    else if (same)
        same = p.ndim <= 1 || p.name.find("temperature") != std::string::npos;
    RF_CHECK_ARG(same, "rf_set_param: size mismatch for %s: got %zu elements in %d dims, expected %zu", name, n, ndim, p.numel());
    RF_CHECK_ARG((reinterpret_cast<uintptr_t>(dev_ptr) & 3) == 0, "rf_set_param: %s is not 4-byte aligned", name);
    p.ptr = dev_ptr;
    h->packed = nullptr;
    return RF_OK;
}

int rf_packed_bytes(const rf_handle* h, size_t* bytes) {
    RF_CHECK_ARG(h && bytes, "rf_packed_bytes: null argument");
    *bytes = h->packed_floats * sizeof(float);
    return RF_OK;
}

int rf_pack_params(rf_handle* h, void* packed_dev, size_t bytes, void* stream) {
    RF_CHECK_ARG(h && packed_dev, "rf_pack_params: null argument");
    RF_CHECK_ARG(aligned16(packed_dev), "rf_pack_params: buffer must be 16-byte aligned");
    if (bytes < h->packed_floats * sizeof(float)) {
        set_error("rf_pack_params: buffer of %zu bytes, need %zu", bytes, h->packed_floats * sizeof(float));
        return RF_E_NOMEM;
    }
    for (const Param& p : h->params)
        if (!p.ptr) {
            set_error("rf_pack_params: missing key '%s'", p.name.c_str());
            return RF_E_MISSING;
        }
    hipStream_t st = (hipStream_t)stream;
    float* base = (float*)packed_dev;
    for (const PackItem& it : h->packs) {
        const Param& p = h->params[it.param];
        int rc;
        if (it.kind == PK_1x1) rc = pack_1x1(p.ptr, base + it.offset, (int)p.shape[0], (int)p.shape[1], p.shape[1], 1, st);
        else if (it.kind == PK_1x1_B3) rc = pack_1x1_b3(p.ptr, base + it.offset, (int)p.shape[0], (int)p.shape[1], p.shape[1], 1, st);
        else if (it.kind == PK_3x3) rc = pack_3x3(p.ptr, base + it.offset, (int)p.shape[0], (int)p.shape[1], st);
        else rc = pack_convT(p.ptr, base + it.offset, (int)p.shape[0], (int)p.shape[1], st);
        if (rc) return rc;
    }
    for (int i = 1; i <= 3; ++i) {
        const int C = h->cfg.dim << (3 - i);
        const std::string u = "up" + std::to_string(i), r = "channel_reduce" + std::to_string(i);
        RF_TRY(pack_upcat(P(h, u + ".weight"), P(h, u + ".bias"), P(h, r + ".weight"), P(h, r + ".bias"), base + h->upcat_offset[i - 1], C, st));
    }
    for (int i = 1; i <= 7; ++i) {
        if (!h->tail_offset[i]) continue;
        const int lvl = i <= 4 ? i - 1 : 7 - i, C = h->cfg.dim << lvl, hc = C * h->cfg.ffn_expansion;
        const std::string pre = "conv_tran" + std::to_string(i) + ".";
        float* composed = base + h->tail_offset[i];
        RF_TRY(pack_tail(P(h, pre + "channel_reduce.weight"), P(h, pre + "channel_reduce.bias"), P(h, pre + "Transformer.ffn.pointwise2.weight"),
                         P(h, pre + "Transformer.ffn.pointwise2.bias"), composed, C, hc, st));
        if (h->tail3_offset[i])
            RF_TRY(launch_tail_fold(P(h, pre + "channel_reduce.weight"), nullptr, composed, base + h->tail3_offset[i], 1, C, hc, st));
    }
    h->packed = base;
    return RF_OK;
}

int rf_workspace_bytes(const rf_handle* h, int B, int H, int W, size_t* bytes) {
    RF_CHECK_ARG(h && bytes, "rf_workspace_bytes: null argument");
    RF_CHECK_ARG(B > 0 && H > 0 && W > 0 && H % 8 == 0 && W % 8 == 0, "packed size %dx%d must be positive multiples of 8 (mosaic divisible by 16)", H, W);
    Plan p;
    RF_TRY(make_plan(h, B, H, W, p));
    *bytes = p.total * sizeof(float);
    return RF_OK;
}

int rf_set_shard(rf_handle* h, int y_lo, int y_hi, int total_rows, rf_allreduce_fn allreduce, void* user) {
    RF_CHECK_ARG(h, "rf_set_shard: null handle");
    if (!allreduce) {
        h->shard_y_lo = h->shard_y_hi = h->shard_total_rows = 0;
        h->shard_allreduce = nullptr; h->shard_user = nullptr;
        return RF_OK;
    }
    RF_CHECK_ARG(h->cfg.variant != RF_VARIANT_TRUECOLOR, "rf_set_shard: variants flca and plain only");
    RF_CHECK_ARG(y_lo >= 0 && y_hi > y_lo && y_lo % 8 == 0 && y_hi % 8 == 0 && total_rows >= y_hi - y_lo && total_rows % 8 == 0,
                 "rf_set_shard: interior rows [%d, %d) of %d must be multiples of 8", y_lo, y_hi, total_rows);
    h->shard_y_lo = y_lo; h->shard_y_hi = y_hi; h->shard_total_rows = total_rows;
    h->shard_allreduce = allreduce; h->shard_user = user;
    return RF_OK;
}

int rf_forward_stage(rf_handle* h, int stage, const float* in, const float* packed, float* out, void* workspace,
                     size_t workspace_bytes, int B, int H, int W, void* stream) {
    RF_CHECK_ARG(h && in && out && workspace && stage >= 1 && stage <= 7, "rf_forward_stage: bad arguments (stage 1..7)");
    RF_CHECK_ARG(B > 0 && B <= 65535 && H > 0 && W > 0 && H % 8 == 0 && W % 8 == 0,
                 "rf_forward_stage: packed size %dx%d must be positive multiples of 8", H, W);
    RF_CHECK_ARG(h->cfg.variant != RF_VARIANT_FLCA || packed, "rf_forward_stage: the FLCA branch needs the packed frame for its guidance");
    RF_CHECK_ARG(h->cfg.variant != RF_VARIANT_TRUECOLOR, "rf_forward_stage: not available for the TrueColor variant");
    if (!h->packed) {
        set_error("rf_forward_stage: parameters not packed (call rf_pack_params after rf_set_param)");
        return RF_E_MISSING;
    }
    RF_CHECK_ARG(aligned16(workspace) && aligned16(in) && aligned16(out), "rf_forward_stage: buffers must be 16-byte aligned");
    Plan p;
    RF_TRY(make_plan(h, B, H, W, p));
    if (workspace_bytes < p.total * sizeof(float)) {
        set_error("rf_forward_stage: workspace of %zu bytes, need %zu", workspace_bytes, p.total * sizeof(float));
        return RF_E_NOMEM;
    }
    hipStream_t st = (hipStream_t)stream;
    float* ws = (float*)workspace;
    const int lvl = stage <= 4 ? stage - 1 : 7 - stage;
    if (h->cfg.variant == RF_VARIANT_FLCA) {
        RF_TRY(launch_guidance_base(packed, 0, h->cfg.clamp_io, ws + p.gscratch, B, H, W, st));
        RF_TRY(launch_guidance_level(ws + p.gscratch, ws + p.guide[lvl], B, H, W, H >> lvl, W >> lvl, st));
    }
    if (p.ks_floats) RF_TRY(check_hip(hipMemsetAsync(ws + p.ks, 0, conv3x3_ksplit_counter_bytes(), st), "rf_forward_stage: memset"));
    return run_stage(h, stage, lvl, in, out, ws, p, B, H, W, st, st);
}

int rf_forward(rf_handle* h, const float* in, float* out, void* workspace, size_t workspace_bytes,
               int B, int H, int W, int packed_input, void* stream) {
    RF_CHECK_ARG(h && in && out && workspace, "rf_forward: null argument");
    RF_CHECK_ARG(B > 0 && B <= 65535 && H > 0 && W > 0 && H % 8 == 0 && W % 8 == 0,
                 "rf_forward: packed size %dx%d must be positive multiples of 8 (mosaic divisible by 16)", H, W);
    RF_CHECK_ARG((size_t)H * W < (1u << 30), "rf_forward: frame too large");
    if (!h->packed) {
        set_error("rf_forward: parameters not packed (call rf_pack_params after rf_set_param)");
        return RF_E_MISSING;
    }
    RF_CHECK_ARG(aligned16(workspace) && aligned16(in) && aligned16(out), "rf_forward: buffers must be 16-byte aligned");
    RF_CHECK_ARG(!h->shard_allreduce || h->shard_y_hi <= H, "rf_forward: shard interior [%d, %d) outside the %d-row window",
                 h->shard_y_lo, h->shard_y_hi, H);
    Plan p;
    RF_TRY(make_plan(h, B, H, W, p));
    if (workspace_bytes < p.total * sizeof(float)) {
        set_error("rf_forward: workspace of %zu bytes, need %zu", workspace_bytes, p.total * sizeof(float));
        return RF_E_NOMEM;
    }
    const rf_config& cfg = h->cfg;
    hipStream_t st = (hipStream_t)stream;
    SideJoinGuard joined(h->side, st);
    float* ws = (float*)workspace;
    const int d = cfg.dim;
    const int mosaic = packed_input ? 0 : 1;

    const int levels = cfg.flca_levels > 0 ? cfg.flca_levels : 2;
    bool use_side = !h->shard_allreduce && cfg.variant != RF_VARIANT_TRUECOLOR;
#ifdef RF_DIAG
    if (getenv("RF_NO_SIDE")) use_side = false;
#endif
    const hipStream_t side = use_side ? h->side.get(st) : st;
    if (p.ks_floats)
        RF_TRY(check_hip(hipMemsetAsync(ws + p.ks, 0, conv3x3_ksplit_counter_bytes(), st), "rf_forward: memset"));
    if (cfg.variant == RF_VARIANT_FLCA) {
        RF_TRY(h->side.fork(st, side));
        RF_TRY(launch_guidance_base(in, mosaic, cfg.clamp_io, ws + p.gscratch, B, H, W, side, h->shard_allreduce, h->shard_user));
        for (int l = 0; l < 4; ++l)
            RF_TRY(launch_guidance_level(ws + p.gscratch, ws + p.guide[l], B, H, W, H >> l, W >> l, side));
    } else if (cfg.variant == RF_VARIANT_TRUECOLOR) {
        const std::string bp = "bayer_processor.";
        RF_TRY(launch_tc_front(in, mosaic, P(h, bp + "wb_gains"), P(h, bp + "color_matrix"),
                               PK(h, bp + "chroma_extractor.0.weight"), P(h, bp + "chroma_extractor.0.bias"),
                               PK(h, bp + "chroma_extractor.2.weight"), P(h, bp + "chroma_extractor.2.bias"),
                               PK(h, bp + "demosaic_refine.0.weight"), P(h, bp + "demosaic_refine.0.bias"),
                               PK(h, bp + "demosaic_refine.2.weight"), P(h, bp + "demosaic_refine.2.bias"),
                               ws + p.gscratch, B, H, W, levels, st));
        for (int l = 0; l < 4; ++l)
            RF_TRY(launch_tc_guide_level(ws + p.gscratch, ws + p.guide[l], B, H, W, levels, H >> l, W >> l, st));
    }
    Conv3x3Args e{};
    e.x = in; e.x_bstride = (int64_t)4 * H * W; e.wp = PK(h, "embedding.weight"); e.bias = P(h, "embedding.bias");
    e.out = ws + p.tA; e.out_bstride = (int64_t)d * H * W; e.B = B; e.Cin = 4; e.Cout = d; e.h = H; e.w = W;
    e.unshuffle_in = mosaic; e.clamp_in = cfg.clamp_io;
    RF_TRY(launch_conv3x3(e, st));

    float* skip[3] = {ws + p.skip[0], ws + p.skip[1], ws + p.skip[2]};
    for (int i = 1; i <= 3; ++i) {
        const int lvl = i - 1, C = d << lvl, hh = H >> lvl, ww = W >> lvl;
        RF_TRY(run_stage(h, i, lvl, ws + p.tA, skip[lvl], ws, p, B, H, W, st, side));
        Conv3x3Args dn{};
        dn.x = skip[lvl]; dn.x_bstride = (int64_t)C * hh * ww; dn.wp = PK(h, "down" + std::to_string(i) + ".body.0.weight");
        dn.out = ws + p.tA; dn.out_bstride = (int64_t)2 * C * (hh / 2) * (ww / 2);
        dn.B = B; dn.Cin = C; dn.Cout = C / 2; dn.h = hh; dn.w = ww; dn.store = 1;
        if (p.ks_floats) { dn.ks_scratch = ws + p.ks; dn.ks_floats = p.ks_floats; }
        RF_TRY(launch_conv3x3(dn, st));
    }
    RF_TRY(run_stage(h, 4, 3, ws + p.tA, ws + p.tB, ws, p, B, H, W, st, side));
    for (int i = 1; i <= 3; ++i) {
        const int lvl = 3 - i, C = d << lvl, hh = H >> lvl, ww = W >> lvl, Pn = hh * ww;
        const std::string u = "up" + std::to_string(i), r = "channel_reduce" + std::to_string(i);
        bool fuse_up = upcat_supported(C, hh / 2, ww / 2, ws + p.tB, skip[lvl], ws + p.tA);
#ifdef RF_DIAG
        if (getenv("RF_NO_UPCAT")) fuse_up = false;
#endif
        if (fuse_up) {
            RF_TRY(launch_upcat(ws + p.tB, skip[lvl], ws + p.tA, h->packed + h->upcat_offset[i - 1], B, C, hh / 2, ww / 2, st));
            RF_TRY(run_stage(h, 4 + i, lvl, ws + p.tA, ws + p.tB, ws, p, B, H, W, st, side));
            continue;
        }
        Conv1x1Args up{};
        up.x1 = ws + p.tB; up.C1 = 2 * C; up.x1_bstride = (int64_t)2 * C * (Pn / 4);
        up.wp = PK(h, u + ".weight"); up.bias = P(h, u + ".bias");
        up.out = ws + p.tU; up.out_bstride = (int64_t)C * Pn; up.Cout = 4 * C; up.B = B; up.P = Pn / 4; up.w = ww / 2; up.mode = 1;
        RF_TRY(launch_conv1x1(up, st));
        Conv1x1Args cr{};
        cr.x1 = ws + p.tU; cr.C1 = C; cr.x1_bstride = (int64_t)C * Pn;
        cr.x2 = skip[lvl]; cr.C2 = C; cr.x2_bstride = (int64_t)C * Pn;
        cr.wp = PK(h, r + ".weight"); cr.bias = P(h, r + ".bias");
        cr.out = ws + p.tA; cr.out_bstride = (int64_t)C * Pn; cr.Cout = C; cr.B = B; cr.P = Pn; cr.w = ww;
        RF_TRY(launch_conv1x1(cr, st));
        RF_TRY(run_stage(h, 4 + i, lvl, ws + p.tA, ws + p.tB, ws, p, B, H, W, st, side));
    }
    Conv3x3Args o{};
    o.x = ws + p.tB; o.x_bstride = (int64_t)d * H * W; o.wp = PK(h, "conv_out.weight"); o.bias = P(h, "conv_out.bias");
    o.out = out; o.out_bstride = (int64_t)cfg.out_channels * 4 * H * W;
    o.B = B; o.Cin = d; o.Cout = 4 * cfg.out_channels; o.h = H; o.w = W; o.act = 1; o.store = 2; o.clamp_out = cfg.clamp_io;
    if (cfg.variant == RF_VARIANT_TRUECOLOR) o.act = 2;
    RF_TRY(launch_conv3x3(o, st));
    if (cfg.variant == RF_VARIANT_TRUECOLOR) {
        const std::string cc = "color_correction.";
        const float* prm[9] = {P(h, cc + "gamma_param"), P(h, cc + "color_transform.0.weight"), P(h, cc + "color_transform.0.bias"),
                               P(h, cc + "color_transform.2.weight"), P(h, cc + "color_transform.2.bias"), P(h, cc + "tone_curve.0.weight"),
                               P(h, cc + "tone_curve.0.bias"), P(h, cc + "tone_curve.2.weight"), P(h, cc + "tone_curve.2.bias")};
        RF_TRY(launch_tc_color_head(out, prm, B, (size_t)4 * H * W, st));
    }
    return RF_OK;
}

}
```

### bayer_low_light_image_enhancement_amd/csrc/rf_pack.hip

```cpp
#include "rf_common.h"

namespace rf {

__global__ void __launch_bounds__(256) pack_1x1_kernel(const float* __restrict__ w, float* __restrict__ packed,
                                                       int Cout, int K, int64_t row_stride, int64_t col_stride) {
    const int NT = (Cout + 15) >> 4, NS = (K + 3) >> 2;
    const size_t total = (size_t)NT * NS * 64;
    for (size_t idx = blockIdx.x * 256ull + threadIdx.x; idx < total; idx += (size_t)gridDim.x * 256) {
        const int l = (int)(idx & 63);
        const int t = (int)((idx >> 6) % NT);
        const int s = (int)((idx >> 6) / NT);
        const int co = 16 * t + (l & 15), k = 4 * s + (l >> 4);
        packed[idx] = (co < Cout && k < K) ? w[co * row_stride + k * col_stride] : 0.f;
    }
}

int pack_1x1(const float* w, float* packed, int Cout, int K, int64_t row_stride, int64_t col_stride, hipStream_t st) {
    const size_t total = packed1x1_floats(K, Cout);
    int g = (int)((total + 255) / 256);
    if (g > 4096) g = 4096;
    pack_1x1_kernel<<<g, 256, 0, st>>>(w, packed, Cout, K, row_stride, col_stride);
    return check_launch("pack_1x1");
}

__global__ void __launch_bounds__(256) pack_1x1_b3_kernel(const float* __restrict__ w, unsigned short* __restrict__ packed3,
                                                          int Cout, int K, int64_t row_stride, int64_t col_stride) {
    const int NT = (Cout + 15) >> 4, NB = (K + 31) >> 5;
    const size_t total = (size_t)NT * NB * 512;
    for (size_t idx = blockIdx.x * 256ull + threadIdx.x; idx < total; idx += (size_t)gridDim.x * 256) {
        const int k = (int)(idx % ((size_t)NB * 32)), co = (int)(idx / ((size_t)NB * 32));
        b3_store(packed3, NT, co, k, (co < Cout && k < K) ? w[co * row_stride + k * col_stride] : 0.f);
    }
}

int pack_1x1_b3(const float* w, void* packed3, int Cout, int K, int64_t row_stride, int64_t col_stride, hipStream_t st) {
    const size_t total = (size_t)cdiv(Cout, 16) * cdiv(K, 32) * 512;
    int g = (int)((total + 255) / 256);
    if (g > 4096) g = 4096;
    pack_1x1_b3_kernel<<<g, 256, 0, st>>>(w, (unsigned short*)packed3, Cout, K, row_stride, col_stride);
    return check_launch("pack_1x1_b3");
}

int pack_convT(const float* w, float* packed, int Cin, int Cout, hipStream_t st) {
    return pack_1x1(w, packed, 4 * Cout, Cin, 1, (int64_t)4 * Cout, st);
}

__global__ void __launch_bounds__(256) pack_3x3_kernel(const float* __restrict__ w, float* __restrict__ packed, int Cout, int Cin) {
    const int NT = (Cout + 15) >> 4, NS = ((Cin + 7) >> 3) * 2;
    const size_t total = (size_t)NS * 18 * NT * 64;
    for (size_t idx = blockIdx.x * 256ull + threadIdx.x; idx < total; idx += (size_t)gridDim.x * 256) {
        const int l = (int)(idx & 63);
        const int t = (int)((idx >> 6) % NT);
        const int e = (int)(((idx >> 6) / NT) % 18);
        const int s = (int)((idx >> 6) / ((size_t)NT * 18));
        const int co = 16 * t + (l & 15), ci = 4 * s + (l >> 4);
        float u = 0.f;
        if (co < Cout && ci < Cin) {
            const float* g = w + ((size_t)co * Cin + ci) * 9 + (e / 6) * 3;
            const int j = e % 6;
            const float s02 = g[0] + g[2];
            const float e02 = fmaf(g[0], 1.0f / 24.0f, g[2] * (1.0f / 6.0f));
            u = j == 0 ? 0.25f * g[0] : j == 1 ? -(s02 + g[1]) * (1.0f / 6.0f) : j == 2 ? -(s02 - g[1]) * (1.0f / 6.0f)
              : j == 3 ? fmaf(g[1], 1.0f / 12.0f, e02) : j == 4 ? fmaf(g[1], -1.0f / 12.0f, e02) : g[2];
        }
        packed[idx] = u;
    }
}

__device__ __forceinline__ size_t pack_item_total(const PackDesc& d) {
    if (d.kind == 0) return (size_t)((d.rows + 15) >> 4) * ((d.cols + 3) >> 2) * 64;
    if (d.kind == 1) return (size_t)(((d.cols + 7) >> 3) * 2) * 18 * ((d.rows + 15) >> 4) * 64;
    if (d.kind == 3) return (size_t)((d.rows + 15) >> 4) * ((d.cols + 31) >> 5) * 512;
    return (size_t)d.rows * 9;
}

__global__ void __launch_bounds__(256) pack_batch_kernel(PackBatch batch) {
    const PackDesc& d = batch.d[blockIdx.y];
    const size_t total = pack_item_total(d);
    const float* __restrict__ w = d.src;
    float* __restrict__ packed = d.dst;
    for (size_t idx = blockIdx.x * 256ull + threadIdx.x; idx < total; idx += (size_t)gridDim.x * 256) {
        if (d.kind == 0) {
            const int NT = (d.rows + 15) >> 4;
            const int l = (int)(idx & 63), t = (int)((idx >> 6) % NT), s = (int)((idx >> 6) / NT);
            const int co = 16 * t + (l & 15), k = 4 * s + (l >> 4);
            packed[idx] = (co < d.rows && k < d.cols) ? w[co * d.rs + k * d.cs] : 0.f;
        } else if (d.kind == 1) {
            const int NT = (d.rows + 15) >> 4;
            const int l = (int)(idx & 63), t = (int)((idx >> 6) % NT), e = (int)(((idx >> 6) / NT) % 18), s = (int)((idx >> 6) / ((size_t)NT * 18));
            const int co = 16 * t + (l & 15), ci = 4 * s + (l >> 4);
            float u = 0.f;
            if (co < d.rows && ci < d.cols) {
                const float* g = w + co * d.rs + ci * d.cs;
                const int dy = e / 6, j = e % 6;
                const float g0 = d.flip ? g[8 - 3 * dy] : g[3 * dy], g1 = d.flip ? g[7 - 3 * dy] : g[3 * dy + 1], g2 = d.flip ? g[6 - 3 * dy] : g[3 * dy + 2];
                const float s02 = g0 + g2;
                const float e02 = fmaf(g0, 1.0f / 24.0f, g2 * (1.0f / 6.0f));
                u = j == 0 ? 0.25f * g0 : j == 1 ? -(s02 + g1) * (1.0f / 6.0f) : j == 2 ? -(s02 - g1) * (1.0f / 6.0f)
                  : j == 3 ? fmaf(g1, 1.0f / 12.0f, e02) : j == 4 ? fmaf(g1, -1.0f / 12.0f, e02) : g2;
            }
            packed[idx] = u;
        } else if (d.kind == 3) {
            const int NT = (d.rows + 15) >> 4, NB = (d.cols + 31) >> 5;
            const int k = (int)(idx % ((size_t)NB * 32)), co = (int)(idx / ((size_t)NB * 32));
            b3_store(reinterpret_cast<unsigned short*>(packed), NT, co, k, (co < d.rows && k < d.cols) ? w[co * d.rs + k * d.cs] : 0.f);
        } else {
            const int t = (int)(idx % 9);
            packed[idx - t + 8 - t] = w[idx];
        }
    }
}

size_t pack_desc_floats(const PackDesc& d) {
    if (d.kind == 0) return packed1x1_floats(d.cols, d.rows);
    if (d.kind == 1) return packed3x3_floats(d.cols, d.rows);
    if (d.kind == 3) return packed1x1_b3_floats(d.cols, d.rows);
    return (size_t)d.rows * 9;
}

int launch_pack_batch(const PackDesc* d, int n, hipStream_t st) {
    for (int i0 = 0; i0 < n; i0 += kPackBatch) {
        PackBatch b;
        const int m = n - i0 < kPackBatch ? n - i0 : kPackBatch;
        size_t biggest = 0;
        for (int i = 0; i < m; ++i) {
            b.d[i] = d[i0 + i];
            const size_t t = pack_desc_floats(d[i0 + i]);
            if (t > biggest) biggest = t;
        }
        int gx = (int)((biggest + 255) / 256);
        if (gx > 256) gx = 256;
        pack_batch_kernel<<<dim3((unsigned)gx, (unsigned)m), 256, 0, st>>>(b);
    }
    return check_launch("pack_batch");
}

int pack_3x3(const float* w, float* packed, int Cout, int Cin, hipStream_t st) {
    const size_t total = packed3x3_floats(Cin, Cout);
    int g = (int)((total + 255) / 256);
    if (g > 4096) g = 4096;
    pack_3x3_kernel<<<g, 256, 0, st>>>(w, packed, Cout, Cin);
    return check_launch("pack_3x3");
}

}
```

Before: 1049 MP/s.

## Add split-bf16 (bf16x3) Winograd 3x3 conv kernel using matrix cores

Adds a new Winograd F(4,3) 3x3 convolution kernel that splits each fp32 value into three bf16 parts and runs the products on bf16 matrix instructions, with weights pre-packed into a new b3 layout. It is used for layers whose Cin is a multiple of 32, and the model now packs and passes these extra weights. The aim is higher matrix throughput than the existing f32 path while keeping close to fp32 accuracy. In exchange it adds packing work, more weight memory and a large new kernel with double-buffered LDS weights and DPP neighbour exchange.

New measurement: 1049 MP/s, median of 4. No clear change (+0.1%).

```diff
diff --git a/bayer_low_light_image_enhancement_amd/build.py b/bayer_low_light_image_enhancement_amd/build.py
--- a/bayer_low_light_image_enhancement_amd/build.py
+++ b/bayer_low_light_image_enhancement_amd/build.py
@@ -11,7 +11,7 @@
 CSRC = os.path.join(HERE, "csrc")
 LIB = os.path.join(CSRC, "librawformer_hip.so")
 DIAG_LIB = os.path.join(CSRC, "librawformer_hip_diag.so")
-DIAG_SOURCES = ["rf_block.hip", "rf_model.hip", "rf_gemm1x1.hip", "rf_fused.hip"]
+DIAG_SOURCES = ["rf_block.hip", "rf_model.hip", "rf_gemm1x1.hip", "rf_fused.hip", "rf_conv3x3.hip"]
 SOURCES = ["rf_api.hip", "rf_model.hip", "rf_pack.hip", "rf_pointwise.hip", "rf_gemm1x1.hip",
            "rf_conv3x3.hip", "rf_attn.hip", "rf_flca.hip", "rf_fused.hip", "rf_block.hip", "rf_harness.hip", "rf_tokattn.hip", "rf_wfb.hip", "rf_upcat.hip", "rf_fft.hip", "rf_ffab.hip", "rf_truecolor.hip", "rf_train.hip", "rf_trainstep.hip"]
 HEADERS = [os.path.join(CSRC, "rf_common.h"), os.path.join(CSRC, "rf_handle.h"), os.path.join(HERE, "..", "include", "rawformer_hip.h"),
diff --git a/bayer_low_light_image_enhancement_amd/csrc/rf_api.hip b/bayer_low_light_image_enhancement_amd/csrc/rf_api.hip
--- a/bayer_low_light_image_enhancement_amd/csrc/rf_api.hip
+++ b/bayer_low_light_image_enhancement_amd/csrc/rf_api.hip
@@ -186,17 +186,19 @@
 
 int rf_conv3x3_scratch_bytes(int Cin, int Cout, size_t* bytes) {
     RF_CHECK_ARG(bytes && Cin > 0 && Cout > 0, "conv3x3_scratch_bytes: bad arguments");
-    *bytes = packed3x3_floats(Cin, Cout) * sizeof(float);
+    *bytes = (align_up(packed3x3_floats(Cin, Cout), 64) + (Cin % 32 == 0 ? packed3x3_b3_floats(Cin, Cout) : 0)) * sizeof(float);
     return RF_OK;
 }
 
 int rf_conv3x3(const float* in, float* out, const float* weight, const float* bias, void* scratch,
                int act, int store, int B, int Cin, int Cout, int h, int w, void* stream) {
-    RF_CHECK_ARG(in && out && weight && scratch && aligned16(scratch), "conv3x3: bad arguments");
+    RF_CHECK_ARG(in && out && weight && scratch && aligned16(scratch) && Cin > 0, "conv3x3: bad arguments");
     hipStream_t st = (hipStream_t)stream;
     RF_TRY(pack_3x3(weight, (float*)scratch, Cout, Cin, st));
+    float* wp3 = Cin % 32 == 0 ? (float*)scratch + align_up(packed3x3_floats(Cin, Cout), 64) : nullptr;
+    if (wp3) RF_TRY(pack_3x3_b3(weight, wp3, Cout, Cin, st));
     Conv3x3Args a{};
-    a.x = in; a.x_bstride = (int64_t)Cin * h * w; a.wp = (const float*)scratch; a.bias = bias;
+    a.x = in; a.x_bstride = (int64_t)Cin * h * w; a.wp = (const float*)scratch; a.wp3 = wp3; a.bias = bias;
     a.out = out; a.out_bstride = (int64_t)Cout * h * w; a.B = B; a.Cin = Cin; a.Cout = Cout; a.h = h; a.w = w;
     a.act = act; a.store = store;
     return launch_conv3x3(a, st);
diff --git a/bayer_low_light_image_enhancement_amd/csrc/rf_common.h b/bayer_low_light_image_enhancement_amd/csrc/rf_common.h
--- a/bayer_low_light_image_enhancement_amd/csrc/rf_common.h
+++ b/bayer_low_light_image_enhancement_amd/csrc/rf_common.h
@@ -55,6 +55,8 @@
 
 static inline size_t packed1x1_b3_floats(int K, int Cout) { return (size_t)cdiv(K, 32) * cdiv(Cout, 16) * 768; }
 int pack_1x1_b3(const float* w, void* packed3, int Cout, int K, int64_t row_stride, int64_t col_stride, hipStream_t st);
+static inline size_t packed3x3_b3_floats(int Cin, int Cout) { return (size_t)cdiv(Cin, 32) * 18 * cdiv(Cout, 16) * 768; }
+int pack_3x3_b3(const float* w, void* packed3, int Cout, int Cin, hipStream_t st);
 #ifdef __HIPCC__
 typedef unsigned u32x4 __attribute__((ext_vector_type(4)));
 typedef __bf16 bf16x8 __attribute__((ext_vector_type(8)));
@@ -166,6 +168,7 @@
     int clamp_out;
     float* ks_scratch = nullptr;
     size_t ks_floats = 0;
+    const void* wp3 = nullptr;
 };
 int launch_conv3x3(const Conv3x3Args& a, hipStream_t st);
 size_t conv3x3_ksplit_floats(int B, int Cout, int h, int w);
diff --git a/bayer_low_light_image_enhancement_amd/csrc/rf_conv3x3.hip b/bayer_low_light_image_enhancement_amd/csrc/rf_conv3x3.hip
--- a/bayer_low_light_image_enhancement_amd/csrc/rf_conv3x3.hip
+++ b/bayer_low_light_image_enhancement_amd/csrc/rf_conv3x3.hip
@@ -6,7 +6,89 @@
 
 static constexpr int KC = 8;
 static constexpr int kKsCounters = 4096;
-typedef unsigned u32x4 __attribute__((ext_vector_type(4)));
+
+__device__ __forceinline__ void wino_output(const f32x4 (&mm)[6], float (&u)[4][4]) {
+#pragma unroll
+    for (int r = 0; r < 4; ++r) {
+        const float s12 = mm[1][r] + mm[2][r], d12 = mm[1][r] - mm[2][r], s34 = mm[3][r] + mm[4][r], d34 = mm[3][r] - mm[4][r];
+        u[r][0] = (mm[0][r] + s12) + s34;
+        u[r][1] = fmaf(2.f, d34, d12);
+        u[r][2] = fmaf(4.f, s34, s12);
+        u[r][3] = fmaf(8.f, d34, d12) + mm[5][r];
+    }
+}
+__device__ __forceinline__ void conv_finish(const Conv3x3Args& a, const float* bias_l, int t, int kq, float (&v)[4][4]) {
+#pragma unroll
+    for (int r = 0; r < 4; ++r) {
+        const float bs = bias_l[16 * t + 4 * kq + r];
+#pragma unroll
+        for (int g = 0; g < 4; ++g) {
+            float u = v[r][g] + bs;
+            if (a.act == 1) u = u > 0.f ? u : 0.2f * u;
+            else if (a.act == 2) u = fmaxf(u, 0.f);
+            else if (a.act == 3) u = gelu_fast(u);
+            else if (a.act == 4) u = 1.0f - 2.0f * __builtin_amdgcn_rcpf(1.0f + __expf(2.0f * u));
+            if (a.clamp_out) u = fminf(fmaxf(u, 0.f), 1.f);
+            v[r][g] = u;
+        }
+    }
+}
+__device__ __forceinline__ void conv_store(const Conv3x3Args& a, float* outb, int cobase, int y, int x, int vec, const float (&v)[4][4]) {
+    const int h = a.h, w = a.w;
+    if (a.store == 0) {
+#pragma unroll
+        for (int r = 0; r < 4; ++r) {
+            const int co = cobase + r;
+            if (co >= a.Cout) continue;
+            float* o = outb + ((size_t)co * h + y) * w + x;
+            if (vec) {
+                *reinterpret_cast<float4*>(o) = make_float4(v[r][0], v[r][1], v[r][2], v[r][3]);
+            } else {
+#pragma unroll
+                for (int g = 0; g < 4; ++g)
+                    if (x + g < w) o[g] = v[r][g];
+            }
+        }
+    } else if (a.store == 1) {
+        const int h2 = h >> 1, w2 = w >> 1;
+#pragma unroll
+        for (int r = 0; r < 4; ++r) {
+            const int co = cobase + r;
+            if (co >= a.Cout) continue;
+            float* o = outb + (((size_t)(4 * co + 2 * (y & 1))) * h2 + (y >> 1)) * w2 + (x >> 1);
+            const size_t ps = (size_t)h2 * w2;
+            if (vec) {
+                *reinterpret_cast<float2*>(o) = make_float2(v[r][0], v[r][2]);
+                *reinterpret_cast<float2*>(o + ps) = make_float2(v[r][1], v[r][3]);
+            } else {
+#pragma unroll
+                for (int g = 0; g < 4; ++g)
+                    if (x + g < w) o[(size_t)(g & 1) * ps + (g >> 1)] = v[r][g];
+            }
+        }
+    } else {
+        if (cobase >= a.Cout) return;
+        const int c = cobase >> 2;
+        float* op = outb + (size_t)c * 4 * h * w;
+        const int w2 = 2 * w;
+        if (vec) {
+#pragma unroll
+            for (int i = 0; i < 2; ++i) {
+                float* row = op + (size_t)(2 * y + i) * w2 + 2 * x;
+                *reinterpret_cast<float4*>(row) = make_float4(v[2 * i][0], v[2 * i + 1][0], v[2 * i][1], v[2 * i + 1][1]);
+                *reinterpret_cast<float4*>(row + 4) = make_float4(v[2 * i][2], v[2 * i + 1][2], v[2 * i][3], v[2 * i + 1][3]);
+            }
+        } else {
+#pragma unroll
+            for (int g = 0; g < 4; ++g)
+                if (x + g < w) {
+#pragma unroll
+                    for (int r = 0; r < 4; ++r)
+                        op[(size_t)(2 * y + (r >> 1)) * w2 + 2 * (x + g) + (r & 1)] = v[r][g];
+                }
+        }
+    }
+}
 
 template <int NCO, int LOG2_RW, int RPW, int NWV, bool KS = false>
 __global__ void __launch_bounds__(64 * NWV, (NWV >= 8 || NCO >= 3) ? 1 : 2) conv3x3_kernel(Conv3x3Args a, int ngroups, int tiles_x, int ntiles, int vec) {
@@ -194,89 +276,6 @@
     int kq_ = kq;
     asm volatile("" : "+v"(kq_));
     const int x = ex0 + 4 * cg;
-    auto transform = [&](int rr, int t, float (&u)[4][4]) {
-        const f32x4* mm = acc[rr][t];
-#pragma unroll
-        for (int r = 0; r < 4; ++r) {
-            const float s12 = mm[1][r] + mm[2][r], d12 = mm[1][r] - mm[2][r], s34 = mm[3][r] + mm[4][r], d34 = mm[3][r] - mm[4][r];
-            u[r][0] = (mm[0][r] + s12) + s34;
-            u[r][1] = fmaf(2.f, d34, d12);
-            u[r][2] = fmaf(4.f, s34, s12);
-            u[r][3] = fmaf(8.f, d34, d12) + mm[5][r];
-        }
-    };
-    auto finish = [&](int t, float (&v)[4][4]) {
-#pragma unroll
-        for (int r = 0; r < 4; ++r) {
-            const float bs = bias_l[16 * t + 4 * kq_ + r];
-#pragma unroll
-            for (int g = 0; g < 4; ++g) {
-                float u = v[r][g] + bs;
-                if (a.act == 1) u = u > 0.f ? u : 0.2f * u;
-                else if (a.act == 2) u = fmaxf(u, 0.f);
-                else if (a.act == 3) u = gelu_fast(u);
-                else if (a.act == 4) u = 1.0f - 2.0f * __builtin_amdgcn_rcpf(1.0f + __expf(2.0f * u));
-                if (a.clamp_out) u = fminf(fmaxf(u, 0.f), 1.f);
-                v[r][g] = u;
-            }
-        }
-    };
-    auto store_tile = [&](int t, int y, const float (&v)[4][4]) {
-        const int cobase = 16 * (t0 + t) + 4 * kq_;
-        if (a.store == 0) {
-#pragma unroll
-            for (int r = 0; r < 4; ++r) {
-                const int co = cobase + r;
-                if (co >= a.Cout) continue;
-                float* o = outb + ((size_t)co * h + y) * w + x;
-                if (vec) {
-                    *reinterpret_cast<float4*>(o) = make_float4(v[r][0], v[r][1], v[r][2], v[r][3]);
-                } else {
-#pragma unroll
-                    for (int g = 0; g < 4; ++g)
-                        if (x + g < w) o[g] = v[r][g];
-                }
-            }
-        } else if (a.store == 1) {
-            const int h2 = h >> 1, w2 = w >> 1;
-#pragma unroll
-            for (int r = 0; r < 4; ++r) {
-                const int co = cobase + r;
-                if (co >= a.Cout) continue;
-                float* o = outb + (((size_t)(4 * co + 2 * (y & 1))) * h2 + (y >> 1)) * w2 + (x >> 1);
-                const size_t ps = (size_t)h2 * w2;
-                if (vec) {
-                    *reinterpret_cast<float2*>(o) = make_float2(v[r][0], v[r][2]);
-                    *reinterpret_cast<float2*>(o + ps) = make_float2(v[r][1], v[r][3]);
-                } else {
-#pragma unroll
-                    for (int g = 0; g < 4; ++g)
-                        if (x + g < w) o[(size_t)(g & 1) * ps + (g >> 1)] = v[r][g];
-                }
-            }
-        } else {
-            if (cobase >= a.Cout) return;
-            const int c = cobase >> 2;
-            float* op = outb + (size_t)c * 4 * h * w;
-            const int w2 = 2 * w;
-            if (vec) {
-#pragma unroll
-                for (int i = 0; i < 2; ++i) {
-                    float* row = op + (size_t)(2 * y + i) * w2 + 2 * x;
-                    *reinterpret_cast<float4*>(row) = make_float4(v[2 * i][0], v[2 * i + 1][0], v[2 * i][1], v[2 * i + 1][1]);
-                    *reinterpret_cast<float4*>(row + 4) = make_float4(v[2 * i][2], v[2 * i + 1][2], v[2 * i][3], v[2 * i + 1][3]);
-                }
-            } else {
-#pragma unroll
-                for (int g = 0; g < 4; ++g)
-                    if (x + g < w) {
-#pragma unroll
-                        for (int r = 0; r < 4; ++r)
-                            op[(size_t)(2 * y + (r >> 1)) * w2 + 2 * (x + g) + (r & 1)] = v[r][g];
-                    }
-            }
-        }
-    };
     if constexpr (!KS) {
 #pragma unroll
         for (int rr = 0; rr < RPW; ++rr) {
@@ -286,9 +285,9 @@
             for (int t = 0; t < NCO; ++t) {
                 if (t0 + t >= NT) break;
                 float v[4][4];
-                transform(rr, t, v);
-                finish(t, v);
-                store_tile(t, y, v);
+                wino_output(acc[rr][t], v);
+                conv_finish(a, bias_l, t, kq_, v);
+                conv_store(a, outb, 16 * (t0 + t) + 4 * kq_, y, x, vec, v);
             }
         }
     } else {
@@ -304,7 +303,7 @@
             for (int t = 0; t < NCO; ++t) {
                 if (t0 + t >= NT) break;
                 float v[4][4];
-                transform(rr, t, v);
+                wino_output(acc[rr][t], v);
 #pragma unroll
                 for (int r = 0; r < 4; ++r) {
                     const int co = 16 * (t0 + t) + 4 * kq_ + r;
@@ -341,12 +340,199 @@
                     }
                     v[r][0] = sum.x; v[r][1] = sum.y; v[r][2] = sum.z; v[r][3] = sum.w;
                 }
-                finish(t, v);
-                store_tile(t, y, v);
+                conv_finish(a, bias_l, t, kq_, v);
+                conv_store(a, outb, 16 * (t0 + t) + 4 * kq_, y, x, vec, v);
             }
         }
         return;
     }
+    }
+}
+
+template <int NCO>
+__global__ void __launch_bounds__(512, 1) conv3x3_b3_kernel(Conv3x3Args a, int ngroups, int tiles_x, int ntiles, int vec) {
+    constexpr int TH = 8, TW = 64;
+    constexpr int SLICE = 6 * NCO * 3 * 64;
+    constexpr int WPT = (SLICE + 511) / 512;
+    constexpr unsigned OOB = 0x80000000u;
+    __shared__ u32x4 lds_w[2 * SLICE];
+    __shared__ float bias_l[NCO * 16];
+
+    const int tid = threadIdx.x;
+    const int lane = tid & 63, wave = tid >> 6;
+    const int j = lane & 15, kq = lane >> 4;
+    const int grp = blockIdx.x % ngroups;
+    const int wg = blockIdx.x / ngroups;
+    const int b = blockIdx.y;
+    const int h = a.h, w = a.w;
+    const int NT = (a.Cout + 15) >> 4;
+    const int t0 = grp * NCO;
+    const int NB = a.Cin >> 5;
+    const float* xb = a.x + (size_t)b * a.x_bstride;
+    const unsigned pb = (unsigned)h * (unsigned)w * 4u;
+    const int step_bytes = 6 * NT * 192 * 16;
+
+    unsigned wvoff[WPT];
+#pragma unroll
+    for (int i = 0; i < WPT; ++i) {
+        const int idx = tid + 512 * i;
+        const int tap = idx / (NCO * 192), r = idx % (NCO * 192);
+        wvoff[i] = idx < SLICE ? (unsigned)(((tap * NT + t0) * 192 + r) * 16) : OOB;
+    }
+    unsigned voff[3], eoff[3];
+    int x0 = 0, y0 = 0;
+    auto plan_tile = [&](int tile) {
+        x0 = (tile % tiles_x) * TW;
+        y0 = (tile / tiles_x) * TH;
+        const int x = x0 + 4 * j;
+        const int xe = j == 0 ? x0 - 1 : x0 + TW;
+        const bool eok = (j == 0 || j == 15) && (unsigned)xe < (unsigned)w;
+#pragma unroll
+        for (int dy = 0; dy < 3; ++dy) {
+            const int y = y0 + wave + dy - 1;
+            const bool yok = (unsigned)y < (unsigned)h;
+            const unsigned row = (unsigned)(8 * kq * h + y) * (unsigned)w;
+            voff[dy] = yok && x < w ? (row + x) * 4u : OOB;
+            eoff[dy] = yok && eok ? (row + xe) * 4u : OOB;
+        }
+    };
+    float4 xr[8];
+    float xe[8];
+    auto load_in = [&](int cb, int dy) {
+        const __amdgpu_buffer_rsrc_t rx = __builtin_amdgcn_make_buffer_rsrc(
+            const_cast<float*>(xb) + (size_t)32 * cb * h * w, 0, cb < NB ? (int)(32u * pb) : 0, 0x00020000);
+#pragma unroll
+        for (int i = 0; i < 8; ++i) {
+            const u32x4 v = __builtin_amdgcn_raw_buffer_load_b128(rx, (int)(voff[dy] + i * pb), 0, 0);
+            xr[i] = make_float4(__uint_as_float(v.x), __uint_as_float(v.y), __uint_as_float(v.z), __uint_as_float(v.w));
+            xe[i] = __uint_as_float(__builtin_amdgcn_raw_buffer_load_b32(rx, (int)(eoff[dy] + i * pb), 0, 0));
+        }
+    };
+    u32x4 win[WPT];
+    auto load_w = [&](int cb, int dy) {
+        const __amdgpu_buffer_rsrc_t rw = __builtin_amdgcn_make_buffer_rsrc(
+            const_cast<u32x4*>(reinterpret_cast<const u32x4*>(a.wp3)) + (size_t)(cb * 18 + dy * 6) * NT * 192, 0, cb < NB ? step_bytes : 0, 0x00020000);
+#pragma unroll
+        for (int i = 0; i < WPT; ++i) win[i] = __builtin_amdgcn_raw_buffer_load_b128(rw, (int)wvoff[i], 0, 0);
+    };
+    auto store_w = [&](int buf) {
+#pragma unroll
+        for (int i = 0; i < WPT; ++i) {
+            const int idx = tid + 512 * i;
+            if (SLICE % 512 == 0 || idx < SLICE) lds_w[buf * SLICE + idx] = win[i];
+        }
+    };
+    auto neighbours = [&](int i, float (&d)[6]) {
+        const float4 v = xr[i];
+        d[0] = __int_as_float(__builtin_amdgcn_update_dpp(__float_as_int(xe[i]), __float_as_int(v.w), 0x111, 0xf, 0xf, false));
+        d[1] = v.x; d[2] = v.y; d[3] = v.z; d[4] = v.w;
+        d[5] = __int_as_float(__builtin_amdgcn_update_dpp(__float_as_int(xe[i]), __float_as_int(v.x), 0x101, 0xf, 0xf, false));
+    };
+    auto wino_in = [](const float (&d)[6], int m) {
+        const float p = fmaf(-4.f, d[2], d[4]), q = fmaf(-4.f, d[1], d[3]);
+        const float c2 = d[4] - d[2], e2 = d[3] - d[1];
+        return m == 0 ? fmaf(4.f, d[0], fmaf(-5.f, d[2], d[4])) : m == 1 ? p + q : m == 2 ? p - q
+             : m == 3 ? fmaf(2.f, e2, c2) : m == 4 ? fmaf(-2.f, e2, c2) : fmaf(4.f, d[1], fmaf(-5.f, d[3], d[5]));
+    };
+
+    f32x4 acc[NCO][6];
+    auto tap_block = [&](const u32x4* lw, int m, const float (&v)[8]) {
+        unsigned p0[8], p1[8], p2[8];
+#pragma unroll
+        for (int i = 0; i < 8; ++i) b3_split(v[i], p0[i], p1[i], p2[i]);
+        u32x4 bq[3];
+        bq[0] = (u32x4){b3_pack(p0[0], p0[1]), b3_pack(p0[2], p0[3]), b3_pack(p0[4], p0[5]), b3_pack(p0[6], p0[7])};
+        bq[1] = (u32x4){b3_pack(p1[0], p1[1]), b3_pack(p1[2], p1[3]), b3_pack(p1[4], p1[5]), b3_pack(p1[6], p1[7])};
+        bq[2] = (u32x4){b3_pack(p2[0], p2[1]), b3_pack(p2[2], p2[3]), b3_pack(p2[4], p2[5]), b3_pack(p2[6], p2[7])};
+        constexpr int TP = NCO < 2 ? NCO : 2;
+#pragma unroll
+        for (int tp = 0; tp < NCO; tp += TP) {
+            u32x4 A[TP][3];
+#pragma unroll
+            for (int u = 0; u < TP; ++u)
+#pragma unroll
+                for (int pc = 0; pc < 3; ++pc) A[u][pc] = lw[((m * NCO + tp + u) * 3 + pc) * 64 + lane];
+#define RF_B3(x) __builtin_bit_cast(bf16x8, x)
+#define RF_B3_TERM(ia, ib)                                                                                                 \
+    _Pragma("unroll") for (int u = 0; u < TP; ++u)                                                                         \
+        acc[tp + u][m] = __builtin_amdgcn_mfma_f32_16x16x32_bf16(RF_B3(A[u][ia]), RF_B3(bq[ib]), acc[tp + u][m], 0, 0, 0);
+            RF_B3_TERM(2, 0) RF_B3_TERM(0, 2) RF_B3_TERM(1, 1) RF_B3_TERM(1, 0) RF_B3_TERM(0, 1) RF_B3_TERM(0, 0)
+#undef RF_B3_TERM
+#undef RF_B3
+        }
+    };
+
+    const int nwg = gridDim.x / ngroups;
+    int tile = wg;
+    if (tile >= ntiles) return;
+    if (tid < NCO * 16) {
+        const int co = 16 * t0 + tid;
+        bias_l[tid] = (a.bias && co < a.Cout) ? a.bias[co] : 0.f;
+    }
+    plan_tile(tile);
+    load_in(0, 0);
+    load_w(0, 0);
+    store_w(0);
+    __syncthreads();
+    int buf = 0;
+    float* outb = a.out + (size_t)b * a.out_bstride;
+    for (; tile < ntiles; tile += nwg) {
+        const int ex0 = x0, ey0 = y0;
+#pragma unroll
+        for (int t = 0; t < NCO; ++t)
+#pragma unroll
+            for (int m = 0; m < 6; ++m) acc[t][m] = (f32x4){0.f, 0.f, 0.f, 0.f};
+        for (int cb = 0; cb < NB; ++cb) {
+#pragma unroll
+            for (int dy = 0; dy < 3; ++dy) {
+                const int ndy = dy < 2 ? dy + 1 : 0;
+                int ncb = dy < 2 ? cb : cb + 1;
+                if (dy == 2 && ncb == NB) {
+                    if (tile + nwg < ntiles) {
+                        plan_tile(tile + nwg);
+                        ncb = 0;
+                    }
+                }
+                const u32x4* lw = lds_w + buf * SLICE;
+                float d[8][6];
+#pragma unroll
+                for (int i = 0; i < 8; ++i) neighbours(i, d[i]);
+                load_w(ncb, ndy);
+#pragma unroll
+                for (int m = 0; m < 3; ++m) {
+                    float v[8];
+#pragma unroll
+                    for (int i = 0; i < 8; ++i) v[i] = wino_in(d[i], m);
+                    tap_block(lw, m, v);
+                }
+                __builtin_amdgcn_sched_barrier(0);
+                store_w(buf ^ 1);
+                float v3[3][8];
+#pragma unroll
+                for (int i = 0; i < 8; ++i)
+#pragma unroll
+                    for (int m = 0; m < 3; ++m) v3[m][i] = wino_in(d[i], m + 3);
+                load_in(ncb, ndy);
+                __builtin_amdgcn_sched_barrier(0);
+#pragma unroll
+                for (int m = 3; m < 6; ++m) tap_block(lw, m, v3[m - 3]);
+                __syncthreads();
+                buf ^= 1;
+            }
+        }
+
+        int kq_ = kq;
+        asm volatile("" : "+v"(kq_));
+        const int x = ex0 + 4 * j, y = ey0 + wave;
+        if (y < h && x < w) {
+#pragma unroll
+            for (int t = 0; t < NCO; ++t) {
+                float v[4][4];
+                wino_output(acc[t], v);
+                conv_finish(a, bias_l, t, kq_, v);
+                conv_store(a, outb, 16 * (t0 + t) + 4 * kq_, y, x, vec, v);
+            }
+        }
     }
 }
 
@@ -367,34 +553,36 @@
     return S;
 }
 
+static dim3 grid_for_tiles(const Conv3x3Args& a, int ntiles, int ngroups) {
+    const long total = (long)ntiles * ngroups * a.B;
+    const int wgs = cdiv(ntiles, (int)((total + 255) / 256));
+    return dim3((unsigned)(ngroups * wgs), (unsigned)a.B);
+}
+
 template <int NCO>
 static void launch_rw(const Conv3x3Args& a, int ngroups, int vec, bool small, hipStream_t st) {
     const int lrw = a.w > 32 ? 0 : (a.w > 16 ? 1 : 2);
     constexpr int RPWB = NCO <= 2 ? 2 : 1;
-    auto grid_for_tiles = [&](int ntiles) {
-        const long total = (long)ntiles * ngroups * a.B;
-        const int wgs = cdiv(ntiles, (int)((total + 255) / 256));
-        return dim3((unsigned)(ngroups * wgs), (unsigned)a.B);
-    };
+    auto grid_for = [&](int ntiles) { return grid_for_tiles(a, ntiles, ngroups); };
     if (small && lrw == 0) {
         const int txs = cdiv(a.w, 64), ntiles = txs * cdiv(a.h, 4);
-        dim3 grid = grid_for_tiles(ntiles);
+        dim3 grid = grid_for(ntiles);
         const int S = ksplit_for(a, ntiles, ngroups, vec, grid);
         grid.z = (unsigned)S;
         if (S > 1) conv3x3_kernel<NCO, 0, 1, 4, true><<<grid, 256, 0, st>>>(a, ngroups, txs, ntiles, vec);
         else conv3x3_kernel<NCO, 0, 1, 4><<<grid, 256, 0, st>>>(a, ngroups, txs, ntiles, vec);
     } else if (NCO == 1 && lrw == 0 && a.h >= 16) {
         const int txs = cdiv(a.w, 64), ntiles = txs * cdiv(a.h, 16);
-        conv3x3_kernel<1, 0, 1, 16><<<grid_for_tiles(ntiles), 1024, 0, st>>>(a, ngroups, txs, ntiles, vec);
+        conv3x3_kernel<1, 0, 1, 16><<<grid_for(ntiles), 1024, 0, st>>>(a, ngroups, txs, ntiles, vec);
     } else if (lrw == 0 && a.h >= 8 * RPWB) {
         const int txs = cdiv(a.w, 64), ntiles = txs * cdiv(a.h, 8 * RPWB);
-        conv3x3_kernel<NCO, 0, RPWB, 8><<<grid_for_tiles(ntiles), 512, 0, st>>>(a, ngroups, txs, ntiles, vec);
+        conv3x3_kernel<NCO, 0, RPWB, 8><<<grid_for(ntiles), 512, 0, st>>>(a, ngroups, txs, ntiles, vec);
     } else if (lrw == 0 && a.h >= 8) {
         const int txs = cdiv(a.w, 64), ntiles = txs * cdiv(a.h, 8);
-        conv3x3_kernel<NCO, 0, 1, 8><<<grid_for_tiles(ntiles), 512, 0, st>>>(a, ngroups, txs, ntiles, vec);
+        conv3x3_kernel<NCO, 0, 1, 8><<<grid_for(ntiles), 512, 0, st>>>(a, ngroups, txs, ntiles, vec);
     } else {
         const int txs = cdiv(a.w, 64 >> lrw), ntiles = txs * cdiv(a.h, 4 << lrw);
-        dim3 grid = grid_for_tiles(ntiles);
+        dim3 grid = grid_for(ntiles);
         const int S = ksplit_for(a, ntiles, ngroups, vec, grid);
         grid.z = (unsigned)S;
         if (S > 1) {
@@ -417,6 +605,7 @@
     int nco = 4;
     if (NT % 4 != 0) nco = (NT % 3 == 0) ? 3 : (NT % 2 == 0 ? 2 : (NT == 1 ? 1 : 4));
     bool small = false;
+    const bool b3_size = a.w > 32 && a.h >= 8 && (long)cdiv(a.w, 64) * cdiv(a.h, nco <= 2 ? 16 : 8) * cdiv(NT, nco) >= 128;
     if (a.w > 32 && a.h >= 8) {
         const long big = (long)cdiv(a.w, 64) * cdiv(a.h, nco <= 2 ? 16 : 8) * cdiv(NT, nco) * a.B;
         if (big < 128) {
@@ -425,9 +614,26 @@
             while (nco > 1 && t4 * cdiv(NT, nco) < 192) nco = (nco == 4 || nco == 2) ? nco / 2 : 1;
         }
     }
+    const int vec = (a.w % 4 == 0) && aligned16(a.out) && (a.out_bstride % 4 == 0);
+    const double px = (double)a.B * a.h * a.w;
+    const double flops = 18.0 * a.Cin * a.Cout * px, bytes = 4.0 * px * (a.Cin + a.Cout);
+    char key[64];
+
+    bool b3 = a.wp3 && aligned16(a.wp3) && a.Cin % 32 == 0 && !a.unshuffle_in && !a.clamp_in && a.w > 32 && a.w % 4 == 0 &&
+              NT % 2 == 0 && b3_size;
+#ifdef RF_DIAG
+    if (getenv("RF_NO_B3")) b3 = false;
+#endif
+    if (b3) {
+        const int ngroups = NT / 2;
+        const int txs = cdiv(a.w, 64), ntiles = txs * cdiv(a.h, 8);
+        const dim3 grid = grid_for_tiles(a, ntiles, ngroups);
+        ProfScope prof(st, "conv3x3_b3_kernel<2>", flops, bytes);
+        conv3x3_b3_kernel<2><<<grid, 512, 0, st>>>(a, ngroups, txs, ntiles, vec);
+        return check_launch("conv3x3_b3");
+    }
+
     const int ngroups = cdiv(NT, nco);
-    const int vec = (a.w % 4 == 0) && aligned16(a.out) && (a.out_bstride % 4 == 0);
-    char key[64];
     {
         const int lrw = a.w > 32 ? 0 : (a.w > 16 ? 1 : 2), rpwb = nco <= 2 ? 2 : 1;
         const int wide = lrw == 0 && a.h >= 8;
@@ -435,8 +641,7 @@
         if (nco == 1 && lrw == 0 && a.h >= 16) snprintf(key, sizeof(key), "conv3x3_kernel<1, 0, 1, 16>");
         if (small) snprintf(key, sizeof(key), "conv3x3_kernel<%d, 0, 1, 4>", nco);
     }
-    const double px = (double)a.B * a.h * a.w;
-    ProfScope prof(st, key, 18.0 * a.Cin * a.Cout * px, 4.0 * px * (a.Cin + a.Cout));
+    ProfScope prof(st, key, flops, bytes);
     switch (nco) {
         case 4: launch_rw<4>(a, ngroups, vec, small, st); break;
         case 3: launch_rw<3>(a, ngroups, vec, small, st); break;
diff --git a/bayer_low_light_image_enhancement_amd/csrc/rf_handle.h b/bayer_low_light_image_enhancement_amd/csrc/rf_handle.h
--- a/bayer_low_light_image_enhancement_amd/csrc/rf_handle.h
+++ b/bayer_low_light_image_enhancement_amd/csrc/rf_handle.h
@@ -16,7 +16,7 @@
     }
 };
 
-enum PackKind { PK_1x1, PK_3x3, PK_CONVT, PK_1x1_B3 };
+enum PackKind { PK_1x1, PK_3x3, PK_CONVT, PK_1x1_B3, PK_3x3_B3 };
 struct PackItem {
     int param;
     PackKind kind;
diff --git a/bayer_low_light_image_enhancement_amd/csrc/rf_model.hip b/bayer_low_light_image_enhancement_amd/csrc/rf_model.hip
--- a/bayer_low_light_image_enhancement_amd/csrc/rf_model.hip
+++ b/bayer_low_light_image_enhancement_amd/csrc/rf_model.hip
@@ -33,10 +33,17 @@
     if (kind == PK_1x1) it.floats = packed1x1_floats((int)p.shape[1], (int)p.shape[0]);
     else if (kind == PK_3x3) it.floats = packed3x3_floats((int)p.shape[1], (int)p.shape[0]);
     else if (kind == PK_1x1_B3) it.floats = packed1x1_b3_floats((int)p.shape[1], (int)p.shape[0]);
+    else if (kind == PK_3x3_B3) it.floats = packed3x3_b3_floats((int)p.shape[1], (int)p.shape[0]);
     else it.floats = packed1x1_floats((int)p.shape[0], 4 * (int)p.shape[1]);
     h->packed_floats += align_up(it.floats, 64);
-    (kind == PK_1x1_B3 ? h->pack3_index : h->pack_index)[name] = (int)h->packs.size();
+    (kind == PK_1x1_B3 || kind == PK_3x3_B3 ? h->pack3_index : h->pack_index)[name] = (int)h->packs.size();
     h->packs.push_back(it);
+}
+
+void add_pack3x3(rf_handle* h, const std::string& name) {
+    add_pack(h, name, PK_3x3);
+    const Param& p = h->params[h->index.at(name)];
+    if (p.shape[1] % 32 == 0 && cdiv((int)p.shape[0], 16) % 2 == 0) add_pack(h, name, PK_3x3_B3);
 }
 
 bool tail_composable(int C, int hc) { return C % 32 == 0 && hc % 32 == 0 && hc > 0; }
@@ -81,7 +88,7 @@
     } else {
         add_param(h, pre + "conv.weight", {C, C, 3, 3});
         add_param(h, pre + "conv.bias", {C});
-        add_pack(h, pre + "conv.weight", PK_3x3);
+        add_pack3x3(h, pre + "conv.weight");
     }
     const std::string t = pre + "Transformer.";
     const int hc = C * cfg.ffn_expansion;
@@ -124,12 +131,16 @@
             h->packed_floats += align_up(packed1x1_b3_floats(2 * C + hc, C), 64);
         }
     }
-    add_pack(h, pre + "Conv_out.weight", PK_3x3);
+    add_pack3x3(h, pre + "Conv_out.weight");
 }
 
 const float* P(const rf_handle* h, const std::string& name) { return h->params[h->index.at(name)].ptr; }
 const float* PK(const rf_handle* h, const std::string& name) { return h->packed + h->packs[h->pack_index.at(name)].offset; }
 const float* PK3(const rf_handle* h, const std::string& name) { return h->packed + h->packs[h->pack3_index.at(name)].offset; }
+const float* PK3_or_null(const rf_handle* h, const std::string& name) {
+    const auto it = h->pack3_index.find(name);
+    return it == h->pack3_index.end() ? nullptr : h->packed + h->packs[it->second].offset;
+}
 
 struct Plan {
     size_t total = 0;
@@ -288,7 +299,8 @@
         r.wp3 = ws + p.wfold_cr3; r.wp3_bstride = (int64_t)packed1x1_b3_floats(compose ? 2 * C + hc : 2 * C, C);
     } else {
         Conv3x3Args cb{};
-        cb.x = in; cb.x_bstride = (int64_t)C * Pn; cb.wp = PK(h, pre + "conv.weight"); cb.bias = P(h, pre + "conv.bias");
+        cb.x = in; cb.x_bstride = (int64_t)C * Pn; cb.wp = PK(h, pre + "conv.weight"); cb.wp3 = PK3_or_null(h, pre + "conv.weight");
+        cb.bias = P(h, pre + "conv.bias");
         cb.out = xs; cb.out_bstride = (int64_t)C * Pn; cb.B = B; cb.Cin = C; cb.Cout = C; cb.h = hh; cb.w = ww;
         cb.act = cfg.branch_lrelu ? 1 : 0;
         RF_TRY(launch_conv3x3(cb, side));
@@ -308,7 +320,8 @@
     RF_TRY(launch_conv1x1(r, st));
 
     Conv3x3Args co{};
-    co.x = crb; co.x_bstride = (int64_t)C * Pn; co.wp = PK(h, pre + "Conv_out.weight"); co.bias = P(h, pre + "Conv_out.bias");
+    co.x = crb; co.x_bstride = (int64_t)C * Pn; co.wp = PK(h, pre + "Conv_out.weight"); co.wp3 = PK3_or_null(h, pre + "Conv_out.weight");
+    co.bias = P(h, pre + "Conv_out.bias");
     co.out = out; co.out_bstride = (int64_t)C * Pn; co.B = B; co.Cin = C; co.Cout = C; co.h = hh; co.w = ww; co.act = 1;
     if (p.ks_floats) { co.ks_scratch = ws + p.ks; co.ks_floats = p.ks_floats; }
     RF_TRY(launch_conv3x3(co, st));
@@ -416,7 +429,7 @@
         add_stage(h, i, C, cfg->heads[i - 1]);
         const std::string n = "down" + std::to_string(i) + ".body.0.weight";
         add_param(h, n, {C / 2, C, 3, 3});
-        add_pack(h, n, PK_3x3);
+        add_pack3x3(h, n);
     }
     add_stage(h, 4, d * 8, cfg->heads[3]);
     for (int i = 1; i <= 3; ++i) {
@@ -434,7 +447,7 @@
     }
     add_param(h, "conv_out.weight", {4 * cfg->out_channels, d, 3, 3});
     add_param(h, "conv_out.bias", {4 * cfg->out_channels});
-    add_pack(h, "conv_out.weight", PK_3x3);
+    add_pack3x3(h, "conv_out.weight");
     if (cfg->variant == RF_VARIANT_TRUECOLOR) {
         add_param(h, "color_correction.gamma_param", {});
         add_param(h, "color_correction.color_transform.0.weight", {64, 3, 1, 1});
@@ -519,6 +532,7 @@
         if (it.kind == PK_1x1) rc = pack_1x1(p.ptr, base + it.offset, (int)p.shape[0], (int)p.shape[1], p.shape[1], 1, st);
         else if (it.kind == PK_1x1_B3) rc = pack_1x1_b3(p.ptr, base + it.offset, (int)p.shape[0], (int)p.shape[1], p.shape[1], 1, st);
         else if (it.kind == PK_3x3) rc = pack_3x3(p.ptr, base + it.offset, (int)p.shape[0], (int)p.shape[1], st);
+        else if (it.kind == PK_3x3_B3) rc = pack_3x3_b3(p.ptr, base + it.offset, (int)p.shape[0], (int)p.shape[1], st);
         else rc = pack_convT(p.ptr, base + it.offset, (int)p.shape[0], (int)p.shape[1], st);
         if (rc) return rc;
     }
@@ -656,6 +670,7 @@
         RF_TRY(run_stage(h, i, lvl, ws + p.tA, skip[lvl], ws, p, B, H, W, st, side));
         Conv3x3Args dn{};
         dn.x = skip[lvl]; dn.x_bstride = (int64_t)C * hh * ww; dn.wp = PK(h, "down" + std::to_string(i) + ".body.0.weight");
+        dn.wp3 = PK3_or_null(h, "down" + std::to_string(i) + ".body.0.weight");
         dn.out = ws + p.tA; dn.out_bstride = (int64_t)2 * C * (hh / 2) * (ww / 2);
         dn.B = B; dn.Cin = C; dn.Cout = C / 2; dn.h = hh; dn.w = ww; dn.store = 1;
         if (p.ks_floats) { dn.ks_scratch = ws + p.ks; dn.ks_floats = p.ks_floats; }
@@ -688,7 +703,8 @@
         RF_TRY(run_stage(h, 4 + i, lvl, ws + p.tA, ws + p.tB, ws, p, B, H, W, st, side));
     }
     Conv3x3Args o{};
-    o.x = ws + p.tB; o.x_bstride = (int64_t)d * H * W; o.wp = PK(h, "conv_out.weight"); o.bias = P(h, "conv_out.bias");
+    o.x = ws + p.tB; o.x_bstride = (int64_t)d * H * W; o.wp = PK(h, "conv_out.weight"); o.wp3 = PK3_or_null(h, "conv_out.weight");
+    o.bias = P(h, "conv_out.bias");
     o.out = out; o.out_bstride = (int64_t)cfg.out_channels * 4 * H * W;
     o.B = B; o.Cin = d; o.Cout = 4 * cfg.out_channels; o.h = H; o.w = W; o.act = 1; o.store = 2; o.clamp_out = cfg.clamp_io;
     if (cfg.variant == RF_VARIANT_TRUECOLOR) o.act = 2;
diff --git a/bayer_low_light_image_enhancement_amd/csrc/rf_pack.hip b/bayer_low_light_image_enhancement_amd/csrc/rf_pack.hip
--- a/bayer_low_light_image_enhancement_amd/csrc/rf_pack.hip
+++ b/bayer_low_light_image_enhancement_amd/csrc/rf_pack.hip
@@ -45,6 +45,13 @@
     return pack_1x1(w, packed, 4 * Cout, Cin, 1, (int64_t)4 * Cout, st);
 }
 
+__device__ __forceinline__ float winograd_tap(const float* g, int j) {
+    const float s02 = g[0] + g[2];
+    const float e02 = fmaf(g[0], 1.0f / 24.0f, g[2] * (1.0f / 6.0f));
+    return j == 0 ? 0.25f * g[0] : j == 1 ? -(s02 + g[1]) * (1.0f / 6.0f) : j == 2 ? -(s02 - g[1]) * (1.0f / 6.0f)
+         : j == 3 ? fmaf(g[1], 1.0f / 12.0f, e02) : j == 4 ? fmaf(g[1], -1.0f / 12.0f, e02) : g[2];
+}
+
 __global__ void __launch_bounds__(256) pack_3x3_kernel(const float* __restrict__ w, float* __restrict__ packed, int Cout, int Cin) {
     const int NT = (Cout + 15) >> 4, NS = ((Cin + 7) >> 3) * 2;
     const size_t total = (size_t)NS * 18 * NT * 64;
@@ -54,17 +61,34 @@
         const int e = (int)(((idx >> 6) / NT) % 18);
         const int s = (int)((idx >> 6) / ((size_t)NT * 18));
         const int co = 16 * t + (l & 15), ci = 4 * s + (l >> 4);
-        float u = 0.f;
-        if (co < Cout && ci < Cin) {
-            const float* g = w + ((size_t)co * Cin + ci) * 9 + (e / 6) * 3;
-            const int j = e % 6;
-            const float s02 = g[0] + g[2];
-            const float e02 = fmaf(g[0], 1.0f / 24.0f, g[2] * (1.0f / 6.0f));
-            u = j == 0 ? 0.25f * g[0] : j == 1 ? -(s02 + g[1]) * (1.0f / 6.0f) : j == 2 ? -(s02 - g[1]) * (1.0f / 6.0f)
-              : j == 3 ? fmaf(g[1], 1.0f / 12.0f, e02) : j == 4 ? fmaf(g[1], -1.0f / 12.0f, e02) : g[2];
-        }
-        packed[idx] = u;
+        packed[idx] = (co < Cout && ci < Cin) ? winograd_tap(w + ((size_t)co * Cin + ci) * 9 + (e / 6) * 3, e % 6) : 0.f;
     }
+}
+
+__global__ void __launch_bounds__(256) pack_3x3_b3_kernel(const float* __restrict__ w, unsigned short* __restrict__ packed3, int Cout, int Cin) {
+    const int NT = (Cout + 15) >> 4, NB = (Cin + 31) >> 5;
+    const size_t total = (size_t)NB * 18 * NT * 512;
+    for (size_t idx = blockIdx.x * 256ull + threadIdx.x; idx < total; idx += (size_t)gridDim.x * 256) {
+        const int k = (int)(idx & 31), row = (int)((idx >> 5) & 15);
+        const size_t et = idx >> 9;
+        const int t = (int)(et % NT);
+        const int e = (int)((et / NT) % 18), s32 = (int)(et / ((size_t)NT * 18));
+        const int co = 16 * t + row, ci = 32 * s32 + k;
+        const float u = (co < Cout && ci < Cin) ? winograd_tap(w + ((size_t)co * Cin + ci) * 9 + (e / 6) * 3, e % 6) : 0.f;
+        unsigned p[3];
+        b3_split(u, p[0], p[1], p[2]);
+        const size_t base = (et * 3 * 64 + row + 16 * (k >> 3)) * 8 + (k & 7);
+#pragma unroll
+        for (int pc = 0; pc < 3; ++pc) packed3[base + (size_t)pc * 512] = (unsigned short)(p[pc] >> 16);
+    }
+}
+
+int pack_3x3_b3(const float* w, void* packed3, int Cout, int Cin, hipStream_t st) {
+    const size_t total = (size_t)cdiv(Cin, 32) * 18 * cdiv(Cout, 16) * 512;
+    int g = (int)((total + 255) / 256);
+    if (g > 4096) g = 4096;
+    pack_3x3_b3_kernel<<<g, 256, 0, st>>>(w, (unsigned short*)packed3, Cout, Cin);
+    return check_launch("pack_3x3_b3");
 }
 
 __device__ __forceinline__ size_t pack_item_total(const PackDesc& d) {
```
